# pxl-th/NNop.jl

Measured on AMD Instinct MI355X. Metric: attention TFLOPs/s + GB/s (fwd, fwd+bwd) at E=64,L=4096,H=4,B=4, higher is better.
Workload: dtype bf16; 1 GPU; C2: bf16 non-causal flash_attention forward, E=64 L=4096 QH=4 KH=4 B=4 per GPU; per_gpu_batch=4, global_batch=4, parallelism=dp1 over (batch, kv-head) slices, step=one nnop_fa_fwd call

## Files before the change

### nnop.jl_amd/csrc/fa_bwd_inst.hpp

```cpp
#pragma once
#include "fa_bwd.hpp"
#include "fa_bwd_w64.hpp"
#include "fa_launch.hpp"
#include "fa_generic.hpp"
#include <math.h>

namespace nnop {

template <typename T, int E> struct BwdCfg {
    static constexpr bool kF32 = sizeof(T) == 4;
    static constexpr int NW_KV = (kF32 && E > 128) ? (NNOP_F32_E256_FORM == 2 ? 4 : NNOP_F32_E256_FORM == 1 ? 2 : 1) : ((kF32 && E > 64 && !fa_bwd_f32_wide<T, E>()) || E > 128) ? 2 : 4;
    static constexpr int BQ    = (kF32 || E > 64) ? 32 : 64;
    static constexpr int NW_Q  = (kF32 && E > 128) ? (NNOP_F32_E256_FORM == 2 ? 4 : 1) : ((kF32 && E > 64 && !fa_bwd_f32_wide<T, E>()) || E > 128) ? 2 : 4;
    static constexpr bool kBig7 = !kF32 && E == 128;
    static constexpr bool kWide8 = !kF32 && E <= 64;
    static constexpr int BK    = (E > 64) ? 32 : 64;
};

static inline int bwd_causal_alt(const nnop_fa_desc& d, long long n_wg, long long cols, int rep, int n_blk, bool pair) {
    if (d.emb > 64 || pair) return 0;
    return causal_alt_run(d.causal != 0, n_wg, cols, rep, n_blk);
}

template <typename T, int E, int NW, int BQ, int MODE, bool WIN = false>
static int launch_dkdv(const nnop_fa_desc& d, const BwdParams& p, hipStream_t s) {
    constexpr int BM = bwd_base_mode(MODE);
    constexpr int lds = fa_bwd_dkdv_lds_bytes<T, E, NW, BQ, BM>() + (BM == 3 ? NW * PairTile<T>::kBytes : 0);
    static_assert(lds <= 160 * 1024, "LDS budget");
    auto kern = fa_bwd_dkdv_kernel<T, E, NW, BQ, MODE, WIN>;
    static unsigned long long lds_done = 0;
    if (ensure_dynamic_lds(kern, lds, &lds_done) != NNOP_OK) return NNOP_ERR_HIP;
    BwdParams pk = p;
    pk.n_blk = (d.kl + 32 * NW - 1) / (32 * NW);
    const long long n_wg = (long long)pk.n_blk * d.kh * d.batch;
    if (n_wg > 0x7fffffffLL) return NNOP_ERR_SHAPE;
    pk.n_wg = (int)n_wg;
    if (n_wg * fa_bwd_split<T, E>() > 0x7fffffffLL) return NNOP_ERR_SHAPE;
    pk.causal_alt = WIN ? 0 : bwd_causal_alt(d, n_wg, (long long)d.kh * d.batch, 1, pk.n_blk, BM >= 2);
    hipLaunchKernelGGL(kern, dim3((unsigned)(n_wg * fa_bwd_split<T, E>())), dim3(NW * 64), lds, s, pk);
    return NNOP_OK;
}

template <typename T, int E, int NW, int BK, int MODE, bool WIN = false>
static int launch_dq(const nnop_fa_desc& d, const BwdParams& p, hipStream_t s) {
    constexpr int BM = bwd_base_mode(MODE);
    constexpr int lds = fa_bwd_dq_lds_bytes<T, E, NW, BK, BM>() + (BM == 3 ? NW * PairTile<T>::kBytes : 0);
    static_assert(lds <= 160 * 1024, "LDS budget");
    auto kern = fa_bwd_dq_kernel<T, E, NW, BK, MODE, WIN>;
    static unsigned long long lds_done = 0;
    if (ensure_dynamic_lds(kern, lds, &lds_done) != NNOP_OK) return NNOP_ERR_HIP;
    BwdParams pq = p;
    pq.n_blk = (d.ql + 32 * NW - 1) / (32 * NW);
    const long long n_wg = (long long)pq.n_blk * d.qh * d.batch;
    if (n_wg > 0x7fffffffLL) return NNOP_ERR_SHAPE;
    pq.n_wg = (int)n_wg;
    if (n_wg * fa_bwd_split<T, E>() > 0x7fffffffLL) return NNOP_ERR_SHAPE;
    pq.causal_alt = WIN ? 0 : bwd_causal_alt(d, n_wg, (long long)d.qh * d.batch, d.qh / d.kh, pq.n_blk, BM >= 2);
    hipLaunchKernelGGL(kern, dim3((unsigned)(n_wg * fa_bwd_split<T, E>())), dim3(NW * 64), lds, s, pq);
    return NNOP_OK;
}

template <typename T, int E, int KIND, int MODE, int NARROW = 0>
static int launch_bwd_w64(const nnop_fa_desc& d, const BwdParams& p, hipStream_t s) {
    using SH = BwdW64Shape<E, KIND, NARROW>;
    constexpr int lds = fa_bwd_w64_lds_bytes<T, E, KIND, NARROW>(MODE != 0);
    static_assert(lds <= 160 * 1024, "LDS budget");
    auto kern = fa_bwd_w64_kernel<T, E, KIND, MODE, NARROW>;
    static unsigned long long lds_done = 0;
    if (ensure_dynamic_lds(kern, lds, &lds_done) != NNOP_OK) return NNOP_ERR_HIP;
    BwdParams pk = p;
    const int len = KIND == kBwdDQ ? d.ql : d.kl, hd = KIND == kBwdDQ ? d.qh : d.kh;
    pk.n_blk = (len + SH::WG_ROWS - 1) / SH::WG_ROWS;
    const long long n_wg = (long long)pk.n_blk * hd * d.batch;
    if (n_wg > 0x7fffffffLL) return NNOP_ERR_SHAPE;
    pk.n_wg = (int)n_wg;
    if (n_wg * SH::NSPLIT > 0x7fffffffLL) return NNOP_ERR_SHAPE;
    long long grid = n_wg * SH::NSPLIT;
    if constexpr (MODE == 1 && SH::NSPLIT == 1) {
        const bool pays = (d.causal && !p.kpad) || (KIND == kBwdDQ && !d.causal && p.kpad && hd % 8 == 0);
        const PersistList l = persist_list((long long)d.batch * hd, hd, pk.n_blk, tune_get(kTuneBwdPersist), pays);
        pk.persist = l.steps;
        pk.persist_hx = l.hx;
        if (l.steps > 0) grid = 256;
    }
    hipLaunchKernelGGL(kern, dim3((unsigned)grid), dim3(256), lds, s, pk);
    return NNOP_OK;
}
static inline bool bwd_w64_ok(const nnop_fa_desc& d, int kind) {
    if (d.dtype == NNOP_F32 || (d.emb != 64 && d.emb != 128 && d.emb != 256)) return false;
    const long long rb = 2LL * d.emb;
    if (kind == kBwdDKDV) {
        if ((long long)(d.qh / d.kh) * d.ql * rb >= (1LL << 32)) return false;
        if ((long long)bwd_rows_padded(d) * 32 >= (1LL << 32)) return false;
        return true;
    }
    return (long long)d.kl * rb < (1LL << 32) && d.kl <= 64 * kMaxMaskTiles;
}
static inline bool bwd_w64_narrow(const nnop_fa_desc& d, int kind) {
    if (d.emb != 64 && d.emb != 128) return false;
    const int knob = tune_get(kTuneBwdNarrow);
    if (knob >= 0) return knob != 0;
    const int len = kind == kBwdDQ ? d.ql : d.kl, hd = kind == kBwdDQ ? d.qh : d.kh;
    return small_grid_prefers_32_row_waves(len, (long long)hd * d.batch, d.causal != 0);
}
static inline int bwd_w64_forms(const nnop_fa_desc& d, bool has_pair, bool ws_aligned16, bool win_on, bool capped) {
    if (has_pair || win_on || capped) return 0;
    const int t = tune_get(kTuneBwdW64);
    const bool want_kv = t < 0 || t == 1 || t == 2 || t == 4, want_q = t < 0 || t == 1 || t == 3 || t == 4;
    return ((want_kv && ws_aligned16 && bwd_w64_ok(d, kBwdDKDV)) ? 1 : 0) | ((want_q && bwd_w64_ok(d, kBwdDQ)) ? 2 : 0);
}

static inline void bwd_params(BwdParams& p, const nnop_fa_desc& d, const BwdArgs& a) {
    p = BwdParams{};
    p.dq = a.dq; p.dk = a.dk; p.dv = a.dv; p.dpair = a.pair ? a.dpair : nullptr;
    p.d_o = a.d_o; p.o = a.o; p.ms = a.ms; p.ls = a.ls;
    p.q = a.q; p.k = a.k; p.v = a.v; p.pair = a.pair; p.kpad = a.kpad;
    p.nl = (float*)a.workspace;
    p.QL = d.ql; p.KL = d.kl; p.QH = d.qh; p.KH = d.kh; p.B = d.batch;
    p.causal = d.causal ? 1 : 0;
    p.scale = (float)(1.0 / sqrt((double)d.emb));
    p.win_left = a.win.left; p.win_right = a.win.right;
    if (a.softcap != 0.f) { const SoftcapK ck = softcap_k(1.0 / sqrt((double)d.emb), a.softcap); p.cap_ka = ck.ka; p.cap_kb = ck.kb; }
}

template <typename T, int E, int MODE, bool WIN = false>
static int launch_bwd_cfg(const nnop_fa_desc& d, const BwdArgs& a, hipStream_t s) {
    using C = BwdCfg<T, E>;
    BwdParams p;
    bwd_params(p, d, a);
    p.QLs = (d.ql + 63) & ~63;
    const long long n_rows = (long long)d.batch * d.qh * p.QLs;
    if (n_rows > 0x7fffffffLL) return NNOP_ERR_SHAPE;
    p.delta = p.nl + n_rows;
    p.rcf = (bwd_has_rcf(d) && ((uintptr_t)a.workspace & 15) == 0) ? (void*)(p.delta + n_rows) : nullptr;
    p.QLp = pair_pad(d.ql); p.KLp = pair_pad(d.kl);
    if constexpr (MODE == 3) {
        const size_t base = (bwd_workspace_bytes(d) + 255) & ~(size_t)255;
        const size_t one = (pair_scratch_elems(d) * sizeof(T) + 255) & ~(size_t)255;
        char* w = (char*)a.workspace + base;
        p.pair_a = w; p.dpair_s = w + one;
        const long long nblk = (long long)d.batch * (p.KLp / 32) * (p.QLp / 32);
        if (nblk > 0x7fffffffLL) return NNOP_ERR_SHAPE;
        PairPackParams pp{a.pair, (void*)p.pair_a, d.ql, d.kl, d.qh, d.batch, p.QLp, p.KLp, d.causal ? 1 : 0};
        hipLaunchKernelGGL((pair_pack_kernel<T>), dim3((unsigned)nblk), dim3(256), 1024 * d.qh * sizeof(T), s, pp);
    }

    const int stages = tune_get(kTuneBwdStages) < 0 ? 7 : tune_get(kTuneBwdStages);
    const int w64_forms = bwd_w64_forms(d, a.pair != nullptr, p.rcf != nullptr, a.win.on(), a.softcap != 0.f);
    const bool w64_kv = (w64_forms & 1) != 0, w64_q = (w64_forms & 2) != 0;
    p.fused = (w64_kv && w64_q && tune_get(kTuneBwdW64) != 4) ? 1 : 0;
    if ((stages & 1) && !p.fused) {
        const long long n_thr = n_rows * (E / 8);
        const long long grid = (n_thr + 255) / 256;
        if (grid > 0x7fffffffLL) return NNOP_ERR_SHAPE;
        hipLaunchKernelGGL((fa_bwd_pre_kernel<T, E>), dim3((unsigned)grid), dim3(256), 0, s, p, n_rows);
    }
    if (p.dpair && MODE != 3) {
        const size_t bytes = (size_t)d.batch * d.kl * d.ql * d.qh * sizeof(T);
        if (hipMemsetAsync(p.dpair, 0, bytes, s) != hipSuccess) { (void)hipGetLastError(); return NNOP_ERR_HIP; }
    }
    const int big_tune = tune_get(kTuneBwdBig7);
    const int big_thr = big_tune >= 0 ? big_tune : (d.causal ? 512 : 256);
    auto run_dkdv = [&]() -> int {
        if constexpr (WIN) return launch_dkdv<T, E, C::NW_KV, C::BQ, MODE, true>(d, p, s);
        else {
        int st = NNOP_OK;
        bool done = false;
        if constexpr (MODE <= 1 && sizeof(T) == 2 && (E == 64 || E == 128 || E == 256)) {
            if (w64_kv) {
                if constexpr (E != 256) {
                    if (bwd_w64_narrow(d, kBwdDKDV)) { st = launch_bwd_w64<T, E, kBwdDKDV, MODE, 1>(d, p, s); done = true; }
                }
                if (!done) { st = launch_bwd_w64<T, E, kBwdDKDV, MODE>(d, p, s); done = true; }
            }
        }
        if constexpr (C::kBig7) if (!done) {
            constexpr int NWB = fa_bwd_dkdv_kregs<T, E, MODE>() ? 8 : 7;
            const long long nb = (long long)((d.kl + 32 * NWB - 1) / (32 * NWB)) * d.kh * d.batch;
            if (nb >= big_thr) { st = launch_dkdv<T, E, NWB, C::BQ, MODE>(d, p, s); done = true; }
        }
        if constexpr (C::kWide8) if (!done) {
            const long long n8 = (long long)((d.kl + 255) / 256) * d.kh * d.batch;
            const int nw = tune_get(kTuneBwdNW);
            if (MODE != 2 && (nw == 8 || nw == 81 || (nw < 0 && !d.causal && n8 >= 256))) { st = launch_dkdv<T, E, 8, C::BQ, MODE>(d, p, s); done = true; }
        }
        if (!done) st = launch_dkdv<T, E, C::NW_KV, C::BQ, MODE>(d, p, s);
        return st;
        }
    };
    auto run_dq = [&]() -> int {
        if constexpr (WIN) return launch_dq<T, E, C::NW_Q, C::BK, MODE, true>(d, p, s);
        else {
        int st = NNOP_OK;
        bool done = false;
        if constexpr (MODE <= 1 && sizeof(T) == 2 && (E == 64 || E == 128 || E == 256)) {
            if (w64_q) {
                if constexpr (E != 256) {
                    if (bwd_w64_narrow(d, kBwdDQ)) {
                        if (MODE == 0 && (d.kl & 63) != 0) st = launch_bwd_w64<T, E, kBwdDQ, 1, 1>(d, p, s);
                        else st = launch_bwd_w64<T, E, kBwdDQ, MODE, 1>(d, p, s);
                        done = true;
                    }
                }
                if (!done) {
                    if (MODE == 0 && (d.kl & 31) != 0) st = launch_bwd_w64<T, E, kBwdDQ, 1>(d, p, s);
                    else st = launch_bwd_w64<T, E, kBwdDQ, MODE>(d, p, s);
                    done = true;
                }
            }
        }
        if constexpr (C::kBig7) if (!done) {
            constexpr int NWB = fa_bwd_dq_qregs<T, E, MODE>() ? 8 : 7;
            const long long nb = (long long)((d.ql + 32 * NWB - 1) / (32 * NWB)) * d.qh * d.batch;
            if (nb >= big_thr) { st = launch_dq<T, E, NWB, C::BK, MODE>(d, p, s); done = true; }
        }
        if constexpr (C::kWide8) if (!done) {
            const long long n8 = (long long)((d.ql + 255) / 256) * d.qh * d.batch;
            const int nw = tune_get(kTuneBwdNW);
            if (MODE != 2 && (nw == 8 || nw == 82 || (nw < 0 && !d.causal && n8 >= 256))) { st = launch_dq<T, E, 8, C::BK, MODE>(d, p, s); done = true; }
        }
        if (!done) st = launch_dq<T, E, C::NW_Q, C::BK, MODE>(d, p, s);
        return st;
        }
    };
    if (p.fused) {
        if (stages & 4) { const int st = run_dq(); if (st != NNOP_OK) return st; }
        if (stages & 2) { const int st = run_dkdv(); if (st != NNOP_OK) return st; }
    } else {
        if (stages & 2) { const int st = run_dkdv(); if (st != NNOP_OK) return st; }
        if (stages & 4) { const int st = run_dq(); if (st != NNOP_OK) return st; }
    }
    if constexpr (MODE == 3) {
        const long long nblk = (long long)d.batch * (p.KLp / 32) * (p.QLp / 32);
        PairUnpackParams up{a.dpair, p.dpair_s, a.kpad, d.ql, d.kl, d.qh, d.batch, p.QLp, p.KLp, d.causal ? 1 : 0,
                            PairTile<T>::kStoreLaneMajor ? 1 : 0};
        hipLaunchKernelGGL((dpair_unpack_kernel<T>), dim3((unsigned)nblk), dim3(256), 1024 * d.qh * sizeof(T), s, up);
    }
    return hipGetLastError() == hipSuccess ? NNOP_OK : NNOP_ERR_HIP;
}

template <typename T, int E>
static int launch_bwd_e(const nnop_fa_desc& d, const BwdArgs& a, hipStream_t s) {
    if (a.softcap != 0.f) {
        if constexpr (sizeof(T) == 4 && E == 256) return NNOP_ERR_EMB_UNSUPPORTED;
        else return a.pair ? launch_bwd_cfg<T, E, 2 | kBwdCap, true>(d, a, s) : launch_bwd_cfg<T, E, 1 | kBwdCap, true>(d, a, s);
    }
    if (a.win.on()) {
        if constexpr (sizeof(T) == 4 && E == 256) {
            if (a.pair) return NNOP_ERR_EMB_UNSUPPORTED;
            return launch_bwd_cfg<T, E, 1, true>(d, a, s);
        } else {
            return a.pair ? launch_bwd_cfg<T, E, 2, true>(d, a, s) : launch_bwd_cfg<T, E, 1, true>(d, a, s);
        }
    }
    if constexpr (sizeof(T) == 4 && E == 256) {
        if (a.pair) return NNOP_ERR_EMB_UNSUPPORTED;
        return (d.causal || a.kpad) ? launch_bwd_cfg<T, E, 1>(d, a, s) : launch_bwd_cfg<T, E, 0>(d, a, s);
    } else
    if (a.pair) {
        if (pair_staged_ok(d) && a.workspace_bytes >= bwd_workspace_bytes_pair(d) && bwd_workspace_bytes_pair(d) > bwd_workspace_bytes(d) &&
            ((uintptr_t)a.workspace & 15) == 0)
            return launch_bwd_cfg<T, E, 3>(d, a, s);
        return launch_bwd_cfg<T, E, 2>(d, a, s);
    }
    if (d.causal || a.kpad) return launch_bwd_cfg<T, E, 1>(d, a, s);
    return launch_bwd_cfg<T, E, 0>(d, a, s);
}

template <typename T> static int launch_bwd_generic(const nnop_fa_desc& d, const BwdArgs& a, hipStream_t s) {
    BwdParams p;
    bwd_params(p, d, a);
    const long long n_rows = (long long)d.batch * d.qh * d.ql, n_krows = (long long)d.batch * d.kh * d.kl;
    p.QLs = d.ql;
    p.delta = p.nl + n_rows;
    const long long gq = (n_rows + 3) / 4, gk = (n_krows + 3) / 4;
    if (gq > 0x7fffffffLL || gk > 0x7fffffffLL) return NNOP_ERR_SHAPE;
    if (p.dpair) {
        const size_t bytes = (size_t)d.batch * d.kl * d.ql * d.qh * sizeof(T);
        if (hipMemsetAsync(p.dpair, 0, bytes, s) != hipSuccess) { (void)hipGetLastError(); return NNOP_ERR_HIP; }
    }
    hipLaunchKernelGGL((fa_bwd_generic_pre_kernel<T>), dim3((unsigned)gq), dim3(256), 0, s, p, d.emb, n_rows);
    const bool cap = a.softcap != 0.f;
    hipLaunchKernelGGL((cap ? fa_bwd_generic_dq_kernel<T, true> : fa_bwd_generic_dq_kernel<T, false>), dim3((unsigned)gq), dim3(256), 0, s, p, d.emb, n_rows);
    hipLaunchKernelGGL((cap ? fa_bwd_generic_dkdv_kernel<T, true> : fa_bwd_generic_dkdv_kernel<T, false>), dim3((unsigned)gk), dim3(256), 0, s, p, d.emb, n_krows);
    return hipGetLastError() == hipSuccess ? NNOP_OK : NNOP_ERR_HIP;
}

template <typename T> int launch_bwd(const nnop_fa_desc& d, const BwdArgs& a, hipStream_t s) {
    if constexpr (sizeof(T) == 2) {
        if (d.emb == 256) return launch_bwd_e<T, 256>(d, a, s);
    } else {
        if (d.emb == 256 && !a.pair && a.softcap == 0.f) return launch_bwd_e<T, 256>(d, a, s);
    }
    if (emb_generic(d.emb)) return launch_bwd_generic<T>(d, a, s);
    switch (d.emb) {
        case 16:  return launch_bwd_e<T, 16>(d, a, s);
        case 32:  return launch_bwd_e<T, 32>(d, a, s);
        case 64:  return launch_bwd_e<T, 64>(d, a, s);
        case 128: return launch_bwd_e<T, 128>(d, a, s);
        default:  return NNOP_ERR_EMB_UNSUPPORTED;
    }
}

}
```

### nnop.jl_amd/csrc/fa_bwd_w64.hpp

```cpp
#pragma once
#include "fa_bwd.hpp"
#include "fa_fwd_w64.hpp"

#if !defined(NNOP_DEV_BUILD)
#undef NNOP_BW64_STAMP
#endif
#ifndef NNOP_BW64_STAMP
#define NNOP_BW64_STAMP 0
#endif
#ifndef NNOP_BW64_LAG
#define NNOP_BW64_LAG 3
#endif
#ifndef NNOP_BW64_PF
#define NNOP_BW64_PF 3
#endif

namespace nnop {

enum : int { kBwdDKDV = 0, kBwdDQ = 1 };

template <typename T, int E> struct DualImg {
    static_assert(sizeof(T) == 2 && (E == 64 || E == 128 || E == 256), "16-bit element types, E = 64, 128 or 256");
    static constexpr int kRowBytes = 2 * E;
    static constexpr int bytes(int rows) { return rows * kRowBytes; }
    NNOP_DEV static constexpr int xor_of(int row) {
        if constexpr (E >= 128) return ((row & 3) << 2) | ((row >> 2) & 3);
        else return (((row >> 1) & 1) << 2) | (((row >> 3) & 1) << 1) | ((row >> 2) & 1);
    }
    NNOP_DEV static int src_of(int o) {
        const int row = o / kRowBytes, phys = (o % kRowBytes) >> 4;
        return row * kRowBytes + ((phys ^ xor_of(row)) << 4);
    }
    NNOP_DEV static int row_lane_base(int lane) {
        const int r = lane & 31, h = lane >> 5;
        return r * kRowBytes + ((xor_of(r) ^ h) << 4);
    }
    NNOP_DEV static int col_lane_base(int lane) {
        const int h = lane >> 5, g1 = (lane >> 4) & 1, q = (lane >> 2) & 3, p = lane & 3;
        const int qx = E >= 128 ? q : (q >> 1);
        return (4 * h + q) * kRowBytes + 16 * (4 * qx + ((2 * g1 + (p >> 1)) ^ h)) + 8 * (p & 1);
    }
};

template <int E, int KIND, int NARROW = 0> struct BwdW64Shape {
    static constexpr bool kDQ = KIND == kBwdDQ;
    static_assert(!NARROW || E == 64 || E == 128, "narrow form: E = 64 / 128");
    static constexpr bool kVLds = !kDQ && E == 128 && !NARROW;
    static constexpr int ZS = (E == 256 || NARROW) ? 1 : ((kDQ || E == 64 || kVLds) ? 2 : 1);
    static constexpr int ZT = E == 256 ? 1 : 2 / ZS;
    static constexpr int NSPLIT = (!kDQ && E == 256) ? 2 : 1;
    static constexpr int NYP = kDQ ? 1 : 2;
    static constexpr int KS = E / 16, EB = E / 32, EBA = EB / NSPLIT;
    static constexpr int NEL = 16 * ZS * ZT;
    static constexpr int RT = 32 * ZT, SW = 32 * ZS, RB = 2 * E;
    static constexpr int IMG = RT * RB;
    static constexpr int RCM = kDQ ? 0 : 1;
    static constexpr int RCB = kDQ ? 0 : RT * 32;
    static constexpr int SLOT = 2 * IMG + RCB, NS = 4;
    static constexpr int NJ = IMG / 4096;
    static constexpr int NPB = 2 * NJ + RCM;
    static constexpr int NFY = NYP * 2 * ZT * EBA, NFX = 2 * ZT * KS, NF = NFY + NFX;
    static constexpr int TB = ZS * (KS + RCM);
    static constexpr int NY = NFY * ZS, NX = 2 * ZT * TB, NSLOT = NY + NX;
    static constexpr int WG_ROWS = 4 * SW;
    static constexpr bool kBases = E == 64 && !kDQ;
    static constexpr int VIMG = kVLds ? WG_ROWS * RB : 0;
    static constexpr int NVB = kVLds ? ZS * KS : 0, PFB = 3, RFB = 4;
    static constexpr int vb_slot(int b) { return NY + TB + ZS * RCM + b; }
    static_assert(IMG % 4096 == 0 && NJ >= 1 && NJ <= 4, "four waves x NJ pieces = one image; 12-bit immediate");
    static_assert(SLOT % (RB > 256 ? RB : 256) == 0, "XOR-addressed fragment reads: slot bases aligned to a row / 256 bytes");
};
template <typename T, int E, int KIND, int NARROW = 0> constexpr int fa_bwd_w64_lds_bytes(bool masked) {
    using SH = BwdW64Shape<E, KIND, NARROW>;
    return SH::NS * SH::SLOT + SH::VIMG + (masked ? (SH::kDQ ? 16 + 8 * kMaxMaskTiles : 16) : 0);
}

template <int E, int KIND, bool MASKED, int LAG, int PF, int NARROW = 0> struct BwdW64Plan {
    using SH = BwdW64Shape<E, KIND, NARROW>;
    static constexpr int NSLOT = SH::NSLOT, NEL = SH::NEL, NITEM = NEL + NEL + NEL / 2;
    static constexpr int BAR_SLOT = (SH::NFY - PF) * SH::ZS;
    int kind[NITEM] = {};
    int el[NITEM] = {};
    int it_end[NSLOT] = {};
    int cost[NSLOT] = {};
    int cap = 0;

    static constexpr bool x_is_rc(int j) { return SH::RCM && (j % SH::TB) / SH::ZS == 0; }
    static constexpr int x_frag(int j) { return (j / SH::TB) * SH::KS + (j % SH::TB) / SH::ZS - SH::RCM; }
    static constexpr int rc_slot(int tq) { return SH::NY + tq * SH::TB; }
    static constexpr int rc_read_slot(int tq) { return rc_slot(tq) - 3 > BAR_SLOT ? rc_slot(tq) - 3 : BAR_SLOT; }
    static constexpr int dma_slot(int d) { return BAR_SLOT + 1 + 2 * d; }
    static constexpr int slot_frag(int s) {
        if (s < SH::NY) return s % SH::ZS == 0 ? s / SH::ZS : -1;
        const int j = s - SH::NY;
        if (x_is_rc(j) || j % SH::ZS != 0) return -1;
        return SH::NFY + x_frag(j);
    }
    static constexpr int pre_cost(int s) {
        int c = 0;
        if (s == BAR_SLOT) c += 8;
        const int f = slot_frag(s % NSLOT);
        if (f >= 0) c += ((f + PF) % SH::NF < SH::NFY ? 24 : 16) + 2 - (SH::kBases ? 4 : 0);
        if (s == NSLOT) c += 24 + 18 + 16 + (MASKED ? 30 : 0);
        return c;
    }
    static constexpr int post_cost(int s) {
        int c = 0;
        for (int tq = 0; tq < 2 * SH::ZT * SH::RCM; ++tq)
            if (s == rc_read_slot(tq)) c += 12;
        if (s == BAR_SLOT + 1) c += SH::kDQ ? 24 : 60;
        if (SH::kBases && s == 1) c += 4 * SH::KS;
        if (SH::kBases && s == SH::NY + 1) c += 8 * SH::EBA;
        for (int b = 0; b < SH::NVB; ++b)
            if (s == SH::vb_slot(b) - SH::PFB) c += 16;
        for (int d = 0; d < SH::NPB; ++d)
            if (s == dma_slot(d)) c += 40 + ((d % SH::NJ == 0 || d >= 2 * SH::NJ) ? 14 : 0);
        return c;
    }
    static constexpr int item_cost(int k) { return k == 0 ? 12 : (k == 1 ? 4 : 4 * SH::NYP); }
    constexpr void list() {
        int n = 0;
        for (int st = 0; st < NEL + LAG; ++st) {
            if (st < NEL) { kind[n] = 0; el[n++] = st; }
            const int m = st - LAG;
            if (m >= 0) {
                kind[n] = 1; el[n++] = m;
                if (m & 1) { kind[n] = 2; el[n++] = m; }
            }
        }
    }
    constexpr bool fill(int budget) {
        int n = 0;
        for (int g = 0; g < NSLOT; ++g) {
            int used = post_cost(g) + pre_cost(g + 1);
            while (n < NITEM && used + item_cost(kind[n]) <= budget && !(g == 0 && kind[n] != 0)) used += item_cost(kind[n++]);
            it_end[g] = n;
            cost[g] = used;
        }
        cap = budget;
        return n == NITEM;
    }
    static constexpr BwdW64Plan make() {
        BwdW64Plan pl{};
        pl.list();
        for (int b = 8; b <= 200; b += 2)
            if (pl.fill(b)) break;
        return pl;
    }
};

template <typename T, int EB> NNOP_DEV void store_acc_row16(T* rowp, f32x16 (&acc)[EB], float mul, int h, bool ok) {
#pragma unroll
    for (int eb = 0; eb < EB; ++eb) {
        acc_after_fence(acc[eb]);
        uint32_t pk[4][2];
#pragma unroll
        for (int g = 0; g < 4; ++g) {
            typedef T t4 __attribute__((ext_vector_type(4)));
            const f32x4 w = {acc[eb][4 * g] * mul, acc[eb][4 * g + 1] * mul, acc[eb][4 * g + 2] * mul, acc[eb][4 * g + 3] * mul};
            const u32x2 u = __builtin_bit_cast(u32x2, __builtin_convertvector(w, t4));
            pk[g][0] = u[0];
            pk[g][1] = u[1];
        }
#pragma unroll
        for (int g = 0; g < 4; g += 2) {
            const auto s0 = __builtin_amdgcn_permlane32_swap(pk[g][0], pk[g + 1][0], false, false);
            const auto s1 = __builtin_amdgcn_permlane32_swap(pk[g][1], pk[g + 1][1], false, false);
            const u32x4 lo = {s0[0], s1[0], s0[1], s1[1]};
            if (ok) *reinterpret_cast<u32x4*>(rowp + 32 * eb + 8 * g + 8 * h) = lo;
        }
    }
}

template <typename T, int E, int KIND, int MODE, int NARROW = 0>
__global__ __launch_bounds__(256, 1) void fa_bwd_w64_kernel(const BwdParams p_arg) {
    using SH = BwdW64Shape<E, KIND, NARROW>;
    using frag_t = typename Elem<T>::frag;
    using Img = DualImg<T, E>;
    using MM = MfmaAsm<T>;
    constexpr bool kDQ = SH::kDQ, kGeneral = MODE != 0;
    constexpr int ZS = SH::ZS, ZT = SH::ZT, NYP = SH::NYP, KS = SH::KS, EB = SH::EBA;
    constexpr int RT = SH::RT, SW = SH::SW, RB = SH::RB, IMG = SH::IMG, SLOT = SH::SLOT, NS = SH::NS, NJ = SH::NJ, NPB = SH::NPB;
    constexpr int NFY = SH::NFY, NF = SH::NF, NY = SH::NY, NX = SH::NX, NSLOT = SH::NSLOT;
    constexpr int PF = NNOP_BW64_PF, RF = 4, LAG = NNOP_BW64_LAG;
    static_assert(NF % RF == 0 && PF < RF && PF < NFY, "static fragment ring; the barrier sits inside phase Y");

    extern __shared__ __attribute__((aligned(16))) char smem[];
#if NNOP_BW64_STAMP
    uint64_t stamp[6];
    stamp[0] = __builtin_amdgcn_s_memtime();
    stamp[1] = __builtin_amdgcn_s_memrealtime();
#endif
    const int wave = __builtin_amdgcn_readfirstlane((int)threadIdx.x >> 6);

    constexpr bool kPersist = kGeneral && SH::NSPLIT == 1;
    const int n_steps_pers = (kPersist && p_arg.persist > 0) ? p_arg.persist : 1;
    for (int pstep = 0; pstep < n_steps_pers; ++pstep) {
    int lane0 = 0;
    if constexpr (kPersist) asm volatile("s_mov_b32 %0, 0" : "=s"(lane0));
    const int lane = kPersist ? (int)__builtin_amdgcn_mbcnt_hi(~0u, __builtin_amdgcn_mbcnt_lo(~0u, (uint32_t)lane0)) : ((int)threadIdx.x & 63);
    const int tid = wave * 64 + lane;
    const int r = lane & 31, h = lane >> 5;
    BwdParams p_blk;
    if constexpr (!kPersist) p_blk = p_arg;
    if constexpr (kPersist) {
        p_blk.dpair = nullptr; p_blk.pair = nullptr; p_blk.pair_a = nullptr; p_blk.dpair_s = nullptr; p_blk.QLp = 0; p_blk.KLp = 0;
        typedef const BwdParams __attribute__((address_space(4))) * params_cp;
        params_cp pp = (params_cp)__builtin_amdgcn_kernarg_segment_ptr();
        asm volatile("" : "+s"(pp));
        p_blk.dq = pp->dq; p_blk.dk = pp->dk; p_blk.dv = pp->dv; p_blk.d_o = pp->d_o; p_blk.o = pp->o; p_blk.ms = pp->ms; p_blk.ls = pp->ls;
        p_blk.q = pp->q; p_blk.k = pp->k; p_blk.v = pp->v; p_blk.kpad = pp->kpad; p_blk.nl = pp->nl; p_blk.delta = pp->delta;
        p_blk.QL = pp->QL; p_blk.KL = pp->KL; p_blk.QH = pp->QH; p_blk.KH = pp->KH; p_blk.B = pp->B; p_blk.causal = pp->causal;
        p_blk.QLs = pp->QLs; p_blk.fused = pp->fused; p_blk.rcf = pp->rcf; p_blk.n_blk = pp->n_blk; p_blk.n_wg = pp->n_wg;
        p_blk.scale = pp->scale; p_blk.persist = pp->persist; p_blk.persist_hx = pp->persist_hx;
    }
    const BwdParams& p = p_blk;
    const float c2 = p.scale * kLog2e;
    const int rep = p.QH / p.KH;
    int pers_col = 0, pers_k = 0;
    if (kPersist && p.persist > 0) {
        const int c = (int)blockIdx.x >> 3;
        const int pos = 32 * pstep + ((pstep & 1) ? 31 - c : c);
        pers_col = pos / p.n_blk;
        pers_k = pos - pers_col * p.n_blk;
    }

    int b, kvh, bh_s;
    int s0wg;
    int SL, TL;
    int heads, u0 = 0, nps;
    if constexpr (kDQ) {
        int blk;
        if (kPersist && p.persist > 0) {
            blk = p.n_blk - 1 - pers_k;
            if (p.persist_hx > 0) bh_s = (pers_col / p.persist_hx) * p.QH + ((int)blockIdx.x & 7) * p.persist_hx + pers_col % p.persist_hx;
            else bh_s = ((int)blockIdx.x & 7) * ((p.B * p.QH) >> 3) + pers_col;
        } else {
            const int lin = xcd_remap_chunked((int)blockIdx.x, p.n_wg, p.n_blk * rep);
            blk = lin % p.n_blk;
            bh_s = lin / p.n_blk;
            if (kGeneral && p.causal) blk = p.n_blk - 1 - blk;
        }
        b = bh_s / p.QH;
        kvh = (bh_s - b * p.QH) / rep;
        s0wg = blk * SH::WG_ROWS;
        SL = p.QL; TL = p.KL; heads = 1;
        nps = (TL + RT - 1) / RT;
        if (kGeneral && p.causal) {
            int last = s0wg + SH::WG_ROWS - 1;
            if (last > SL - 1) last = SL - 1;
            const int t_c = last / RT + 1;
            if (t_c < nps) nps = t_c;
        }
    } else {
        int blk;
        if (kPersist && p.persist > 0) {
            blk = pers_k;
            if (p.persist_hx > 0) bh_s = (pers_col / p.persist_hx) * p.KH + ((int)blockIdx.x & 7) * p.persist_hx + pers_col % p.persist_hx;
            else bh_s = ((int)blockIdx.x & 7) * ((p.B * p.KH) >> 3) + pers_col;
        } else {
            const int lin = xcd_remap_chunked((int)blockIdx.x % p.n_wg, p.n_wg, p.n_blk);
            blk = lin % p.n_blk;
            bh_s = lin / p.n_blk;
        }
        b = bh_s / p.KH;
        kvh = bh_s - b * p.KH;
        s0wg = blk * SH::WG_ROWS;
        SL = p.KL; TL = p.QL; heads = rep;
        const int nst = (TL + RT - 1) / RT;
        if (kGeneral && p.causal) u0 = s0wg / RT < nst ? s0wg / RT : nst;
        nps = nst - u0;
    }
    const int esplit = SH::NSPLIT > 1 ? (int)blockIdx.x / p.n_wg : 0;
    const int s0w = s0wg + wave * SW;
    int sidx[ZS], sidx_c[ZS];
#pragma unroll
    for (int zs = 0; zs < ZS; ++zs) {
        sidx[zs] = s0w + 32 * zs + r;
        sidx_c[zs] = sidx[zs] < SL ? sidx[zs] : SL - 1;
    }

    const T* __restrict__ b1p;
    const T* __restrict__ b2p;
    const char* __restrict__ t1p;
    const char* __restrict__ t2p;
    uint32_t t_bytes;
    if constexpr (kDQ) {
        b1p = (const T*)p.q + (size_t)bh_s * p.QL * E;
        b2p = (const T*)p.d_o + (size_t)bh_s * p.QL * E;
        t1p = (const char*)((const T*)p.k + (size_t)(b * p.KH + kvh) * p.KL * E);
        t2p = (const char*)((const T*)p.v + (size_t)(b * p.KH + kvh) * p.KL * E);
        t_bytes = (uint32_t)p.KL * (uint32_t)RB;
    } else {
        b1p = (const T*)p.k + (size_t)bh_s * p.KL * E;
        b2p = (const T*)p.v + (size_t)bh_s * p.KL * E;
        const size_t g0 = (size_t)(b * p.QH + kvh * rep) * p.QL * E;
        t1p = (const char*)((const T*)p.q + g0);
        t2p = (const char*)((const T*)p.d_o + g0);
        t_bytes = (uint32_t)rep * (uint32_t)p.QL * (uint32_t)RB;
    }
    const int U = heads * nps;

    const uint8_t* __restrict__ mp = kGeneral && p.kpad ? p.kpad + (size_t)b * p.KL : nullptr;
    bool svalid[ZS];
#pragma unroll
    for (int zs = 0; zs < ZS; ++zs) svalid[zs] = sidx[zs] < SL;
    uint64_t* const vbits = reinterpret_cast<uint64_t*>(smem + NS * SLOT + SH::VIMG + 16);
    int n_steps = U;
    if constexpr (kGeneral && !kDQ) {
        if (mp) {
            bool any = false;
#pragma unroll
            for (int zs = 0; zs < ZS; ++zs) {
                if (svalid[zs]) svalid[zs] = mp[sidx[zs]] != 0;
                any = any || svalid[zs];
            }
            int* flag = reinterpret_cast<int*>(smem + NS * SLOT + SH::VIMG);
            if (tid == 0) *flag = 0;
            __syncthreads();
            if (any) *flag = 1;
            __syncthreads();
            if (*flag == 0) n_steps = 0;
        }
    }
    if constexpr (kGeneral && kDQ) {
        int* slot = reinterpret_cast<int*>(smem + NS * SLOT + SH::VIMG);
        const int nk = n_steps * RT < p.KL ? n_steps * RT : p.KL;
        if (mp) {
            const int last = kpad_scan(mp, p.KL, nk, vbits, kMaxMaskTiles, slot, tid, 256);
            const int t_m = last / RT + 1;
            if (t_m < n_steps) n_steps = t_m;
        } else {
            for (int w = tid; w * 64 < nk; w += 256) {
                const int left = p.KL - w * 64;
                vbits[w] = left >= 64 ? ~0ull : ((1ull << left) - 1ull);
            }
            __syncthreads();
        }
    }

    n_steps = __builtin_amdgcn_readfirstlane(n_steps);

    float rc_nl[ZS], rc_nd[ZS];
    frag_t rc_do[kDQ ? ZS : 1][kDQ ? KS : 1], rc_o[kDQ ? ZS : 1][kDQ ? KS : 1];
    T rc_m[ZS], rc_l[ZS];
    if constexpr (kDQ) {
#pragma unroll
        for (int zs = 0; zs < ZS; ++zs) {
            const bool in = sidx[zs] < SL;
            const size_t row = (size_t)bh_s * p.QL + sidx_c[zs];
            const T* drow = (const T*)p.d_o + row * E;
#pragma unroll
            for (int ks = 0; ks < KS; ++ks) rc_do[zs][ks] = *reinterpret_cast<const frag_t*>(drow + 16 * ks + 8 * h);
            if (p.fused) {
                const T* orow = (const T*)p.o + row * E;
#pragma unroll
                for (int ks = 0; ks < KS; ++ks) rc_o[zs][ks] = *reinterpret_cast<const frag_t*>(orow + 16 * ks + 8 * h);
                rc_m[zs] = ((const T*)p.ms)[row];
                rc_l[zs] = ((const T*)p.ls)[row];
            } else {
                const size_t ro = (size_t)bh_s * p.QLs + sidx_c[zs];
                rc_nl[zs] = in ? p.nl[ro] : -INFINITY;
                rc_nd[zs] = in ? p.delta[ro] : 0.f;
            }
        }
    }
    auto finish_rc = [&]() {
        if constexpr (kDQ) {
            if (!p.fused) return;
#pragma unroll
            for (int zs = 0; zs < ZS; ++zs) {
                float part = 0.f;
#pragma unroll
                for (int ks = 0; ks < KS; ++ks)
#pragma unroll
                    for (int j = 0; j < 8; ++j) part += to_f32(rc_do[zs][ks][j]) * to_f32(rc_o[zs][ks][j]);
                const float dl = half_swap_sum(part);
                const float m = to_f32(rc_m[zs]), l = to_f32(rc_l[zs]);
                float nlv = -(m * kLog2e + __builtin_amdgcn_logf(l)) / c2;
                float ndv = -dl;
                if (!(l > 0.f) || !(nlv == nlv) || m == -INFINITY) { nlv = -INFINITY; ndv = 0.f; }
                if (!(sidx[zs] < SL)) { nlv = -INFINITY; ndv = 0.f; }
                if (p.rcf && sidx[zs] < p.QLs && h == 0) {
                    typedef T t8 __attribute__((ext_vector_type(8)));
                    t8* dst = reinterpret_cast<t8*>(p.rcf) + 2 * ((size_t)bh_s * p.QLs + sidx[zs]);
                    dst[0] = rc_split3<T>(nlv);
                    dst[1] = rc_split3<T>(ndv);
                }
                rc_nl[zs] = nlv;
                rc_nd[zs] = ndv;
            }
        }
    };
    if (n_steps == 0) finish_rc();
    f32x16 acc[NYP][ZS][EB];
#pragma unroll
    for (int y = 0; y < NYP; ++y)
#pragma unroll
        for (int zs = 0; zs < ZS; ++zs)
#pragma unroll
            for (int eb = 0; eb < EB; ++eb) {
#pragma unroll
                for (int i = 0; i < 16; ++i) acc[y][zs][eb][i] = 0.f;
                asm volatile("" : "+a"(acc[y][zs][eb]));
            }

    if (n_steps > 0) {
        const uint32_t lds0 = (uint32_t)(uintptr_t)smem;
        if ((TL & (RT - 1)) != 0) {
            for (int i = tid * 16; i < NS * SLOT; i += 256 * 16) *reinterpret_cast<u32x4*>(smem + i) = u32x4{0, 0, 0, 0};
            __syncthreads();
        }
        uint32_t voff[NJ];
#pragma unroll
        for (int j = 0; j < NJ; ++j) voff[j] = (uint32_t)(Img::src_of((wave * NJ + j) * 1024 + lane * 16) - j * 1024);
        const uint32_t wave_off = (uint32_t)(wave * NJ * 1024);
        const u32x4 rs1 = make_rsrc(t1p, t_bytes), rs2 = make_rsrc(t2p, t_bytes);
        u32x4 rsc = rs1;
        uint32_t rc_voff = 0;
        if constexpr (!kDQ) {
            rsc = make_rsrc(p.rcf, (uint32_t)((size_t)p.B * p.QH * p.QLs * 32));
            rc_voff = (uint32_t)lane * 16u + (uint32_t)((wave % (RT / 32)) * 1024);
        }
        const uint32_t rc_dst_off = (uint32_t)(2 * IMG) + (uint32_t)((wave % (RT / 32 > 0 ? RT / 32 : 1)) * 1024);
        int d_s = 0;
        uint32_t d_off = (uint32_t)u0 * (uint32_t)(RT * RB);
        uint32_t d_rc = kDQ ? 0u : ((uint32_t)(b * p.QH + kvh * rep) * (uint32_t)p.QLs + (uint32_t)(u0 * RT)) * 32u;
        const uint32_t jump_off = ((uint32_t)p.QL - (uint32_t)((nps - 1) * RT)) * (uint32_t)RB;
        const uint32_t jump_rc = ((uint32_t)p.QLs - (uint32_t)((nps - 1) * RT)) * 32u;
        auto advance_dma = [&]() {
            if constexpr (kDQ) {
                d_off += (uint32_t)(RT * RB);
            } else {
                const int s1 = d_s + 1;
                const bool wrap = s1 == nps;
                d_s = wrap ? 0 : s1;
                d_off += wrap ? jump_off : (uint32_t)(RT * RB);
                d_rc += wrap ? jump_rc : (uint32_t)(RT * 32);
            }
        };
        auto issue_step = [&](uint32_t slot) {
            static_for<NJ>([&](auto jc) { constexpr int j = decltype(jc)::value; dma_piece<j, j == 0>(rs1, voff[j], d_off, slot); });
            static_for<NJ>([&](auto jc) { constexpr int j = decltype(jc)::value; dma_piece<j, j == 0>(rs2, voff[j], d_off, slot + IMG); });
            if constexpr (!kDQ) dma_piece<0, true>(rsc, rc_voff, d_rc, slot - wave_off + rc_dst_off);
        };
        uint32_t sM = lds0 + wave_off, sX = sM + SLOT, sF = sM + 2 * SLOT, sD = sM + 3 * SLOT, sY = sM;
        auto rotate_slots = [&]() { sY = sM; sM = sX; sX = sF; sF = sD; sD = sY; };

        constexpr bool kVLds = SH::kVLds;
        frag_t b1[ZS][KS], b2[kVLds ? 1 : ZS][kVLds ? 1 : KS];
#pragma unroll
        for (int zs = 0; zs < ZS; ++zs)
#pragma unroll
            for (int ks = 0; ks < KS; ++ks) {
                if constexpr (kVLds) {
                    b1[zs][ks] = *reinterpret_cast<const frag_t*>(b1p + (size_t)sidx_c[zs] * E + 16 * ks + 8 * h);
                } else {
                    b1[zs][ks] = load_q_frag<frag_t>(b1p + (size_t)sidx_c[zs] * E + 16 * ks + 8 * h);
                    if constexpr (kDQ) b2[zs][ks] = rc_do[zs][ks];
                    else b2[zs][ks] = load_q_frag<frag_t>(b2p + (size_t)sidx_c[zs] * E + 16 * ks + 8 * h);
                }
            }
        const uint32_t vimg0 = lds0 + (uint32_t)(NS * SLOT);
        if constexpr (kVLds) {
            const u32x4 rsv = make_rsrc(b2p, (uint32_t)SL * (uint32_t)RB);
            const uint32_t vsoff = (uint32_t)s0wg * (uint32_t)RB;
            static_for<16>([&](auto jc) {
                constexpr int j = decltype(jc)::value;
                const uint32_t vo = (uint32_t)(Img::src_of((wave * 16 + j) * 1024 + lane * 16) - (j & 3) * 1024);
                dma_piece<(j & 3), (j & 3) == 0>(rsv, vo, vsoff, vimg0 + (uint32_t)(wave * 16384 + (j >> 2) * 4096));
            });
        }
        issue_step(sM);
        advance_dma();
        issue_step(sX);
        advance_dma();
        issue_step(sF);
        advance_dma();
        finish_rc();
        float nl2[ZS];
        f32x16 ndl[ZS];
        if constexpr (kDQ) {
#pragma unroll
            for (int zs = 0; zs < ZS; ++zs) {
                nl2[zs] = rc_nl[zs] * c2;
#pragma unroll
                for (int i = 0; i < 16; ++i) ndl[zs][i] = rc_nd[zs];
            }
            if constexpr (ZS == 2) fence_valu_operand(ndl[0], ndl[1]);
            else asm volatile("s_nop 1" : "+v"(ndl[0]));
        }
        constexpr bool kBonesV = E == 256 || kVLds;
        frag_t bones;
        if constexpr (!kDQ) {
#pragma unroll
            for (int j = 0; j < 8; ++j) bones[j] = from_f32<T>((h == 0 && j < 3) ? 1.0f : 0.0f);
            if constexpr (kBonesV) asm volatile("s_nop 1" : "+v"(bones));
            else asm volatile("s_nop 1" : "+a"(bones));
        }
        auto rc_tile = [&](frag_t rc) -> f32x16 { if constexpr (kBonesV) return MM::qk_first_v(rc, bones); else return MM::qk_first(rc, bones); };

        f32x16 sA[ZS][ZT], dA[ZS][ZT], sB[ZS][ZT], dB[ZS][ZT];
        u32x4 fA[NYP][ZS][2 * ZT], fB[NYP][ZS][2 * ZT];
#pragma unroll
        for (int y = 0; y < NYP; ++y)
#pragma unroll
            for (int zs = 0; zs < ZS; ++zs)
#pragma unroll
                for (int kk = 0; kk < 2 * ZT; ++kk) { fA[y][zs][kk] = u32x4{0, 0, 0, 0}; fB[y][zs][kk] = u32x4{0, 0, 0, 0}; }

        typedef __attribute__((address_space(3))) const frag_t* lds_frag_p;
        typedef __attribute__((address_space(3))) s16x4* lds_tr_p;
        const uint32_t row_lane = (uint32_t)Img::row_lane_base(lane) - wave_off;
        const uint32_t col_lane = (uint32_t)Img::col_lane_base(lane) + (uint32_t)(esplit * EB * 64) - wave_off;
        const uint32_t rc_lane0 = (uint32_t)(2 * IMG + r * 32 + 16 * h) - wave_off;
        const uint32_t rc_lane1 = (uint32_t)(2 * IMG + r * 32 + 16) - wave_off;
        auto opaque = [](uint32_t x) { asm volatile("" : "+v"(x)); return x; };
        auto pin = [](auto& x) { asm volatile("" : "+v"(x)); };
        auto read_row = [&](uint32_t ra, int g) -> frag_t {
            const int prod = g / (ZT * KS), zt = (g / KS) % ZT, ks = g % KS;
            return *(lds_frag_p)(uintptr_t)((ra ^ (uint32_t)(ks << 5)) + (uint32_t)(prod * IMG + zt * 32 * RB));
        };
        auto read_col = [&](uint32_t ca, int f) -> frag_t {
            const int y = f / (2 * ZT * EB), kk = (f / EB) % (2 * ZT), eb = f % EB;
            const int img = kDQ ? 0 : (y == 0 ? IMG : 0);
            const s16x4 a = __builtin_amdgcn_ds_read_tr16_b64_v4i16((lds_tr_p)(uintptr_t)((ca ^ (uint32_t)(eb << 6)) + (uint32_t)(img + 16 * kk * RB)));
            const s16x4 c = __builtin_amdgcn_ds_read_tr16_b64_v4i16((lds_tr_p)(uintptr_t)((ca ^ (uint32_t)((eb << 6) | 32)) + (uint32_t)(img + (16 * kk + 8) * RB)));
            typedef short s16x8 __attribute__((ext_vector_type(8)));
            const s16x8 v8 = {a[0], a[1], a[2], a[3], c[0], c[1], c[2], c[3]};
            return __builtin_bit_cast(frag_t, v8);
        };
        auto read_row_b = [&](const uint32_t (&rb)[KS], int g) -> frag_t {
            const int prod = g / (ZT * KS), zt = (g / KS) % ZT, ks = g % KS;
            return *(lds_frag_p)(uintptr_t)(rb[ks] + (uint32_t)(prod * IMG + zt * 32 * RB));
        };
        auto read_col_b = [&](const uint32_t (&cb)[2 * EB], int f) -> frag_t {
            const int y = f / (2 * ZT * EB), kk = (f / EB) % (2 * ZT), eb = f % EB;
            const int img = kDQ ? 0 : (y == 0 ? IMG : 0);
            const s16x4 a = __builtin_amdgcn_ds_read_tr16_b64_v4i16((lds_tr_p)(uintptr_t)(cb[2 * eb] + (uint32_t)(img + 16 * kk * RB)));
            const s16x4 c = __builtin_amdgcn_ds_read_tr16_b64_v4i16((lds_tr_p)(uintptr_t)(cb[2 * eb + 1] + (uint32_t)(img + (16 * kk + 8) * RB)));
            typedef short s16x8 __attribute__((ext_vector_type(8)));
            const s16x8 v8 = {a[0], a[1], a[2], a[3], c[0], c[1], c[2], c[3]};
            return __builtin_bit_cast(frag_t, v8);
        };
        const uint32_t v_lane = vimg0 + (uint32_t)(wave * 64 * RB + Img::row_lane_base(lane));
        auto read_vb = [&](int b) -> frag_t {
            const int ks = b / ZS, zs = b % ZS;
            return *(lds_frag_p)(uintptr_t)((v_lane ^ (uint32_t)(ks << 5)) + (uint32_t)(zs * 32 * RB));
        };
        auto read_rcf = [&](uint32_t rca, int zt) -> frag_t { return *(lds_frag_p)(uintptr_t)(rca + (uint32_t)(zt * 1024)); };

        uint64_t vword_next = 0;
        auto vword_fetch = [&](int u) { const int w = (u * RT) >> 6; vword_next = vbits[w < kMaxMaskTiles ? w : kMaxMaskTiles - 1]; };
        using vword_t = std::conditional_t<(kDQ && RT == 64), uint64_t, uint32_t>;
        constexpr vword_t kAllValid = ~(vword_t)0;
        auto vword_take = [&](int u) -> vword_t {
            const uint64_t w = ((uint64_t)(uint32_t)__builtin_amdgcn_readfirstlane((uint32_t)(vword_next >> 32)) << 32) |
                               (uint64_t)(uint32_t)__builtin_amdgcn_readfirstlane((uint32_t)vword_next);
            return (vword_t)(w >> ((u * RT) & 63));
        };
        auto apply_mask = [&](f32x16 (&s)[ZS][ZT], int t0, vword_t valid) {
#pragma unroll
            for (int zs = 0; zs < ZS; ++zs)
#pragma unroll
                for (int zt = 0; zt < ZT; ++zt) {
                    uint32_t m;
                    if constexpr (kDQ) {
                        const int lim = (p.causal ? sidx[zs] : 0x3fffffff) - t0 - 32 * zt - 4 * h;
                        const uint32_t cm = lim >= 31 ? ~0u : (lim < 0 ? 0u : ((2u << lim) - 1u));
                        m = (uint32_t)(valid >> (32 * zt + 4 * h)) & cm;
                    } else {
                        const int lim = sidx[zs] - t0 - 32 * zt - 4 * h;
                        m = lim <= 0 ? ~0u : (lim >= 32 ? 0u : ~((1u << lim) - 1u));
                    }
#pragma unroll
                    for (int i = 0; i < 16; ++i) {
                        const int lr = (i & 3) + 8 * (i >> 2);
                        s[zs][zt][i] = ((m >> lr) & 1u) ? s[zs][zt][i] : -INFINITY;
                    }
                }
        };
        int c_s = 0;
        auto step_t0 = [&]() -> int { return (u0 + c_s) * RT; };
        auto step_needs_mask = [&](int t0, vword_t valid) -> bool {
            if constexpr (kDQ) return valid != kAllValid || (p.causal && t0 + RT - 1 > s0w);
            else return p.causal && t0 < s0w + SW - 1;
        };

        if constexpr (kVLds) {
#pragma unroll
            for (int zs = 0; zs < ZS; ++zs)
#pragma unroll
                for (int ks = 0; ks < KS; ++ks) landed(b1[zs][ks]);
            asm volatile("s_waitcnt vmcnt(%c[nfl])\n\ts_barrier" :: [nfl] "n"(2 * NPB) : "memory");
        } else if constexpr (KS == 16) {
            static_assert(ZS == 1, "");
            asm volatile("s_waitcnt vmcnt(%c[nfl])\n\ts_barrier"
                         : "+a"(b1[0][0]), "+a"(b1[0][1]), "+a"(b1[0][2]), "+a"(b1[0][3]), "+a"(b1[0][4]), "+a"(b1[0][5]), "+a"(b1[0][6]), "+a"(b1[0][7])
                         : [nfl] "n"(2 * NPB) : "memory");
            asm volatile("" : "+a"(b1[0][8]), "+a"(b1[0][9]), "+a"(b1[0][10]), "+a"(b1[0][11]), "+a"(b1[0][12]), "+a"(b1[0][13]), "+a"(b1[0][14]), "+a"(b1[0][15]) :: "memory");
            asm volatile("" : "+a"(b2[0][0]), "+a"(b2[0][1]), "+a"(b2[0][2]), "+a"(b2[0][3]), "+a"(b2[0][4]), "+a"(b2[0][5]), "+a"(b2[0][6]), "+a"(b2[0][7]) :: "memory");
            asm volatile("" : "+a"(b2[0][8]), "+a"(b2[0][9]), "+a"(b2[0][10]), "+a"(b2[0][11]), "+a"(b2[0][12]), "+a"(b2[0][13]), "+a"(b2[0][14]), "+a"(b2[0][15]) :: "memory");
        } else if constexpr (KS == 8 && ZS == 2) {
            asm volatile("s_waitcnt vmcnt(%c[nfl])\n\ts_barrier"
                         : "+a"(b1[0][0]), "+a"(b1[0][1]), "+a"(b1[0][2]), "+a"(b1[0][3]), "+a"(b1[0][4]), "+a"(b1[0][5]), "+a"(b1[0][6]), "+a"(b1[0][7]),
                           "+a"(b1[1][0]), "+a"(b1[1][1]), "+a"(b1[1][2]), "+a"(b1[1][3]), "+a"(b1[1][4]), "+a"(b1[1][5]), "+a"(b1[1][6]), "+a"(b1[1][7])
                         : [nfl] "n"(2 * NPB) : "memory");
            asm volatile(""
                         : "+a"(b2[0][0]), "+a"(b2[0][1]), "+a"(b2[0][2]), "+a"(b2[0][3]), "+a"(b2[0][4]), "+a"(b2[0][5]), "+a"(b2[0][6]), "+a"(b2[0][7]),
                           "+a"(b2[1][0]), "+a"(b2[1][1]), "+a"(b2[1][2]), "+a"(b2[1][3]), "+a"(b2[1][4]), "+a"(b2[1][5]), "+a"(b2[1][6]), "+a"(b2[1][7])
                         :: "memory");
        } else if constexpr (KS == 8) {
            asm volatile("s_waitcnt vmcnt(%c[nfl])\n\ts_barrier"
                         : "+a"(b1[0][0]), "+a"(b1[0][1]), "+a"(b1[0][2]), "+a"(b1[0][3]), "+a"(b1[0][4]), "+a"(b1[0][5]), "+a"(b1[0][6]), "+a"(b1[0][7]),
                           "+a"(b2[0][0]), "+a"(b2[0][1]), "+a"(b2[0][2]), "+a"(b2[0][3]), "+a"(b2[0][4]), "+a"(b2[0][5]), "+a"(b2[0][6]), "+a"(b2[0][7])
                         : [nfl] "n"(2 * NPB) : "memory");
        } else if constexpr (KS == 4 && ZS == 1) {
            asm volatile("s_waitcnt vmcnt(%c[nfl])\n\ts_barrier"
                         : "+a"(b1[0][0]), "+a"(b1[0][1]), "+a"(b1[0][2]), "+a"(b1[0][3]), "+a"(b2[0][0]), "+a"(b2[0][1]), "+a"(b2[0][2]), "+a"(b2[0][3])
                         : [nfl] "n"(2 * NPB) : "memory");
        } else {
            static_assert(KS == 4 && ZS == 2, "");
            asm volatile("s_waitcnt vmcnt(%c[nfl])\n\ts_barrier"
                         : "+a"(b1[0][0]), "+a"(b1[0][1]), "+a"(b1[0][2]), "+a"(b1[0][3]), "+a"(b1[1][0]), "+a"(b1[1][1]), "+a"(b1[1][2]), "+a"(b1[1][3]),
                           "+a"(b2[0][0]), "+a"(b2[0][1]), "+a"(b2[0][2]), "+a"(b2[0][3]), "+a"(b2[1][0]), "+a"(b2[1][1]), "+a"(b2[1][2]), "+a"(b2[1][3])
                         : [nfl] "n"(2 * NPB) : "memory");
        }

        {
            const uint32_t ra = opaque(sM + row_lane);
            const uint32_t rca[2] = {opaque(sM + rc_lane0), opaque(sM + rc_lane1)};
#pragma unroll
            for (int prod = 0; prod < 2; ++prod)
#pragma unroll
                for (int zt = 0; zt < ZT; ++zt) {
                    if constexpr (!kDQ) {
                        const frag_t rc = read_rcf(rca[prod], zt);
#pragma unroll
                        for (int zs = 0; zs < ZS; ++zs) (prod ? dA : sA)[zs][zt] = rc_tile(rc);
                    }
#pragma unroll
                    for (int ks = 0; ks < KS; ++ks) {
                        const frag_t a = read_row(ra, (prod * ZT + zt) * KS + ks);
#pragma unroll
                        for (int zs = 0; zs < ZS; ++zs) {
                            f32x16& d = (prod ? dA : sA)[zs][zt];
                            if constexpr (kVLds) {
                                const frag_t bq = prod ? read_vb(ks * ZS + zs) : b1[zs][ks];
                                MM::qk_acc_v(d, a, bq);
                            } else {
                                const frag_t& bq = (prod ? b2 : b1)[zs][ks];
                                if (kDQ && ks == 0) d = prod ? MM::qk_init(a, bq, ndl[zs]) : MM::qk_first(a, bq);
                                else MM::qk_acc(d, a, bq);
                            }
                        }
                    }
                }
            if constexpr (ZS == 2) {
                fence_mfma_result(sA[0][0], sA[1][0], dA[0][0], dA[1][0]);
            } else if constexpr (ZT == 2) {
                fence_mfma_result(sA[0][0], sA[0][1], dA[0][0], dA[0][1]);
            } else {
                asm volatile(NNOP_FENCE_128 : "+v"(sA[0][0]), "+v"(dA[0][0]));
            }
        }
        if constexpr (kGeneral && kDQ) vword_fetch(0);

        frag_t fr[RF];
        {
            const uint32_t ca0 = opaque(sY + col_lane);
#pragma unroll
            for (int f = 0; f < PF; ++f) fr[f] = read_col(ca0, f);
        }

        constexpr bool kBases = SH::kBases;
        uint32_t cbase[2 * EB], rbase[KS];
        auto set_cbase = [&](uint32_t slot) {
            const uint32_t ca = opaque(slot + col_lane);
#pragma unroll
            for (int j = 0; j < 2 * EB; ++j) { cbase[j] = ca ^ (uint32_t)(((j >> 1) << 6) | ((j & 1) << 5)); pin(cbase[j]); }
        };
        if constexpr (kBases) set_cbase(sY);

        using Plan = BwdW64Plan<E, KIND, kGeneral, LAG, PF, NARROW>;
        auto iteration = [&](int u, f32x16 (&sc)[ZS][ZT], f32x16 (&dc)[ZS][ZT], f32x16 (&sn)[ZS][ZT], f32x16 (&dn)[ZS][ZT],
                             u32x4 (&fw)[NYP][ZS][2 * ZT], u32x4 (&fp)[NYP][ZS][2 * ZT]) {
            constexpr Plan plan = Plan::make();
            static_assert(plan.it_end[NSLOT - 1] == Plan::NITEM, "every item placed");
            static_assert(Plan::dma_slot(NPB - 1) < NSLOT, "the DMA batch fits behind the barrier");
            if constexpr (kGeneral) {
                const int t0 = step_t0();
                vword_t valid = kAllValid;
                if constexpr (kDQ) {
                    valid = vword_take(u);
                    vword_fetch(u + 1);
                }
                if (__builtin_expect(step_needs_mask(t0, valid), 0)) apply_mask(sc, t0, valid);
            }
            const uint32_t cimg = opaque(sY + col_lane);
            const uint32_t cimg2 = opaque(sM + col_lane);
            const uint32_t rimg = opaque(sX + row_lane);
            uint32_t rcimg[2] = {0, 0};
            if constexpr (!kDQ) { rcimg[0] = opaque(sX + rc_lane0); rcimg[1] = opaque(sX + rc_lane1); }
            frag_t rcf[2 * ZT];
            frag_t vb[kVLds ? SH::RFB : 1];
            uint32_t dst = 0, soff = 0, srow = 0;

            auto item = [&](auto kc) {
                constexpr int k = decltype(kc)::value, kind = plan.kind[k], n = plan.el[k];
                constexpr int t = n >> 4, zs = ZS == 2 ? t : 0, zt = ZS == 2 ? 0 : t, i = n & 15;
                if constexpr (kind == 0) {
                    float x;
                    if constexpr (kDQ) x = __builtin_fmaf(sc[zs][zt][i], c2, nl2[zs]);
                    else x = sc[zs][zt][i] * c2;
                    float e = fast_exp2(x);
                    pin(e);
                    sc[zs][zt][i] = e;
                } else if constexpr (kind == 1) {
                    float ds = sc[zs][zt][i] * dc[zs][zt][i];
                    pin(ds);
                    dc[zs][zt][i] = ds;
                } else {
                    typedef T t2 __attribute__((ext_vector_type(2)));
                    constexpr int kk = 2 * zt + (i >> 3), w = (i & 7) >> 1;
                    if constexpr (!kDQ) {
                        const f32x2 pw = {sc[zs][zt][i - 1], sc[zs][zt][i]};
                        uint32_t word2 = __builtin_bit_cast(uint32_t, __builtin_convertvector(pw, t2));
                        pin(word2);
                        fw[0][zs][kk][w] = word2;
                    }
                    const f32x2 dsw = {dc[zs][zt][i - 1], dc[zs][zt][i]};
                    uint32_t word = __builtin_bit_cast(uint32_t, __builtin_convertvector(dsw, t2));
                    pin(word);
                    fw[NYP - 1][zs][kk][w] = word;
                }
            };
            auto movable = [&](auto sc_) {
                constexpr int sl = decltype(sc_)::value;
                constexpr int k0 = sl ? plan.it_end[sl - 1] : 0, k1 = plan.it_end[sl];
                static_for<k1 - k0>([&](auto dk_) { item(std::integral_constant<int, k0 + decltype(dk_)::value>{}); });
            };
            auto read_ahead = [&](auto fc) {
                constexpr int g = decltype(fc)::value + PF;
                if constexpr (kBases) {
                    if constexpr (g < NFY) fr[g % RF] = read_col_b(cbase, g);
                    else if constexpr (g < NF) fr[g % RF] = read_row_b(rbase, g - NFY);
                    else fr[g % RF] = read_col_b(cbase, g - NF);
                } else {
                    if constexpr (g < NFY) fr[g % RF] = read_col(cimg, g);
                    else if constexpr (g < NF) fr[g % RF] = read_row(rimg, g - NFY);
                    else fr[g % RF] = read_col(cimg2, g - NF);
                }
            };

            static_for<NSLOT>([&](auto ic) {
                constexpr int i = decltype(ic)::value;
                constexpr int f = Plan::slot_frag(i);
                if constexpr (i == Plan::BAR_SLOT) {
                    static_assert(NPB <= 15, "vmcnt literal");
                    asm volatile("s_waitcnt vmcnt(%0)\n\ts_barrier" :: "n"(NPB) : "memory");
                }
                if constexpr (f >= 0) read_ahead(std::integral_constant<int, f>{});
                if constexpr (i < NY) {
                    constexpr int fy = i / ZS, zs = i % ZS;
                    constexpr int y = fy / (2 * ZT * EB), kk = (fy / EB) % (2 * ZT), eb = fy % EB;
                    MM::pv_acc(acc[y][zs][eb], fr[fy % RF], __builtin_bit_cast(frag_t, fp[y][zs][kk]));
                } else {
                    constexpr int j = i - NY, tq = j / SH::TB, prod = tq / ZT, zt = tq % ZT, zs = (j % SH::TB) % ZS;
                    f32x16& d = (prod ? dn : sn)[zs][zt];
                    if constexpr (Plan::x_is_rc(j)) {
                        d = rc_tile(rcf[tq]);
                    } else {
                        constexpr int g = Plan::x_frag(j), ks = g % KS;
                        if constexpr (kVLds) {
                            if constexpr (prod == 0) MM::qk_acc_v(d, fr[(NFY + g) % RF], b1[zs][ks]);
                            else MM::qk_acc_v(d, fr[(NFY + g) % RF], vb[(ks * ZS + zs) % SH::RFB]);
                        } else {
                            const frag_t& bq = (prod ? b2 : b1)[zs][ks];
                            if constexpr (kDQ && ks == 0) d = prod ? MM::qk_init(fr[(NFY + g) % RF], bq, ndl[zs]) : MM::qk_first(fr[(NFY + g) % RF], bq);
                            else MM::qk_acc(d, fr[(NFY + g) % RF], bq);
                        }
                    }
                }
                __builtin_amdgcn_sched_barrier(0);
                if constexpr (!kDQ) {
                    static_for<2 * ZT>([&](auto tc) {
                        constexpr int tq = decltype(tc)::value;
                        if constexpr (i == Plan::rc_read_slot(tq)) rcf[tq] = read_rcf(rcimg[tq / ZT], tq % ZT);
                    });
                }
                if constexpr (kVLds) {
                    static_for<SH::NVB>([&](auto bc) {
                        constexpr int b = decltype(bc)::value;
                        if constexpr (i == SH::vb_slot(b) - SH::PFB) vb[b % SH::RFB] = read_vb(b);
                    });
                }
                if constexpr (kBases && i == 1) {
#pragma unroll
                    for (int ks = 0; ks < KS; ++ks) { rbase[ks] = rimg ^ (uint32_t)(ks << 5); pin(rbase[ks]); }
                }
                if constexpr (kBases && i == NY + 1) set_cbase(sM);
                if constexpr (i == Plan::BAR_SLOT + 1) {
                    dst = sD;
                    soff = d_off;
                    srow = d_rc;
                    advance_dma();
                    asm volatile("" : "+s"(d_off));
                }
                static_for<NPB>([&](auto dc_) {
                    constexpr int d = decltype(dc_)::value;
                    if constexpr (i == Plan::dma_slot(d)) {
                        if constexpr (d < NJ) dma_piece<d, d == 0>(rs1, voff[d < NJ ? d : 0], soff, dst);
                        else if constexpr (d < 2 * NJ) dma_piece<d - NJ, d == NJ>(rs2, voff[d < 2 * NJ ? d - NJ : 0], soff, dst + IMG);
                        else dma_piece<0, true>(rsc, rc_voff, srow, dst - wave_off + rc_dst_off);
                    }
                });
                movable(std::integral_constant<int, i>{});
                __builtin_amdgcn_sched_barrier(0);
            });
            rotate_slots();
            if constexpr (kGeneral) {
                if constexpr (kDQ) ++c_s;
                else { if (++c_s == nps) c_s = 0; }
            }
        };

        auto leave_fence = []() { asm volatile(NNOP_FENCE_128 ::: "memory"); __builtin_amdgcn_sched_barrier(0); };
#if NNOP_BW64_STAMP
        stamp[2] = __builtin_amdgcn_s_memtime();
        stamp[3] = __builtin_amdgcn_s_memrealtime();
#endif
        int n_live = n_steps;
        if constexpr (kDQ && kGeneral) {
            if (p.causal) {
                const int t_w = (s0w + SW - 1) / RT + 1;
                if (t_w < n_live) n_live = t_w;
            }
        }
        int u = 0;
        const int n_it = n_live + 1;
        if (n_it >= 2) {
            for (;;) {
                iteration(u, sA, dA, sB, dB, fA, fB);
                iteration(u + 1, sB, dB, sA, dA, fB, fA);
                u += 2;
                if (u + 1 >= n_it) {
                    leave_fence();
                    break;
                }
            }
        }
        if (u < n_it) {
            iteration(u, sA, dA, sB, dB, fA, fB);
            leave_fence();
            ++u;
        }
        if constexpr (kDQ && kGeneral) {
            for (; u <= n_steps; ++u) {
                asm volatile("s_waitcnt vmcnt(%0)\n\ts_barrier" :: "n"(NPB) : "memory");
                issue_step(sD);
                advance_dma();
                rotate_slots();
            }
        }
        asm volatile("s_waitcnt vmcnt(0)" ::: "memory");
#if NNOP_BW64_STAMP
        stamp[4] = __builtin_amdgcn_s_memtime();
        stamp[5] = __builtin_amdgcn_s_memrealtime();
#endif
    }

    fence_acc_result(acc[0][0][0]);
    int lane1 = 0;
    if constexpr (kPersist) asm volatile("s_mov_b32 %0, 0" : "=s"(lane1));
    const int lane_e = kPersist ? (int)__builtin_amdgcn_mbcnt_hi(~0u, __builtin_amdgcn_mbcnt_lo(~0u, (uint32_t)lane1)) : lane;
    const int h_e = lane_e >> 5;
#pragma unroll
    for (int zs = 0; zs < ZS; ++zs) {
        const int sidx_e = kPersist ? s0w + 32 * zs + (lane_e & 31) : sidx[zs];
        const int sidx_ce = sidx_e < SL ? sidx_e : SL - 1;
        const bool in = sidx_e < SL;
        if constexpr (kDQ) {
            T* row = (T*)p.dq + ((size_t)bh_s * p.QL + sidx_ce) * E + esplit * EB * 32;
            store_acc_row16<T, EB>(row, acc[0][zs], p.scale, h_e, in);
        } else {
            if constexpr (kGeneral) {
                if (!svalid[zs]) {
#pragma unroll
                    for (int y = 0; y < NYP; ++y)
#pragma unroll
                        for (int eb = 0; eb < EB; ++eb) {
                            acc_after_fence(acc[y][zs][eb]);
#pragma unroll
                            for (int i = 0; i < 16; ++i) acc[y][zs][eb][i] = 0.f;
                        }
                }
            }
            const size_t ro = ((size_t)bh_s * p.KL + sidx_ce) * E + esplit * EB * 32;
            store_acc_row16<T, EB>((T*)p.dv + ro, acc[0][zs], 1.0f, h_e, in);
            store_acc_row16<T, EB>((T*)p.dk + ro, acc[1][zs], p.scale, h_e, in);
        }
    }
#if NNOP_BW64_STAMP
    if (tid == 0) {
        uint64_t* dbg = kDQ ? reinterpret_cast<uint64_t*>((T*)p.dq + ((size_t)bh_s * p.QL + s0w) * E)
                            : reinterpret_cast<uint64_t*>((T*)p.dk + ((size_t)bh_s * p.KL + s0w) * E);
        for (int i = 0; i < 6; ++i) dbg[i] = stamp[i];
        dbg[6] = (uint64_t)n_steps;
    }
#endif
    if (pstep + 1 < n_steps_pers) __syncthreads();
    }
}

}
```

Baseline: 984.8 TFLOP/s.

## Use compile-time LDS ring slots and an MHA-specialised dK/dV backward kernel

Turns the four-slot LDS ring of the w64 backward kernel from rotating runtime registers into compile-time slot indices. The main loop is unrolled four times so fragment reads and buffer-to-LDS DMA can use immediate offsets from precomputed per-lane base registers. Adds a one-head variant for the dK/dV pass when query heads equal kv heads, which removes the per-step wrap logic, and retunes the scheduling cost model. The aim is fewer address computations and scalar ALU work per step, at the cost of more code size and register pressure.

```diff
diff --git a/nnop.jl_amd/csrc/fa_bwd_inst.hpp b/nnop.jl_amd/csrc/fa_bwd_inst.hpp
--- a/nnop.jl_amd/csrc/fa_bwd_inst.hpp
+++ b/nnop.jl_amd/csrc/fa_bwd_inst.hpp
@@ -60,12 +60,18 @@
     return NNOP_OK;
 }
 
-template <typename T, int E, int KIND, int MODE, int NARROW = 0>
+template <typename T, int E, int KIND, int MODE, int NARROW = 0, bool ONEHEAD = false>
 static int launch_bwd_w64(const nnop_fa_desc& d, const BwdParams& p, hipStream_t s) {
     using SH = BwdW64Shape<E, KIND, NARROW>;
+    if constexpr (!ONEHEAD && KIND == kBwdDKDV && E == 64 && NARROW == 0) {
+        if (d.qh == d.kh) return launch_bwd_w64<T, E, KIND, MODE, NARROW, true>(d, p, s);
+    }
     constexpr int lds = fa_bwd_w64_lds_bytes<T, E, KIND, NARROW>(MODE != 0);
     static_assert(lds <= 160 * 1024, "LDS budget");
-    auto kern = fa_bwd_w64_kernel<T, E, KIND, MODE, NARROW>;
+    auto kern = [] {
+        if constexpr (ONEHEAD) return fa_bwd_w64_mha_kernel<T, E, KIND, MODE, NARROW>;
+        else return fa_bwd_w64_kernel<T, E, KIND, MODE, NARROW>;
+    }();
     static unsigned long long lds_done = 0;
     if (ensure_dynamic_lds(kern, lds, &lds_done) != NNOP_OK) return NNOP_ERR_HIP;
     BwdParams pk = p;
diff --git a/nnop.jl_amd/csrc/fa_bwd_w64.hpp b/nnop.jl_amd/csrc/fa_bwd_w64.hpp
--- a/nnop.jl_amd/csrc/fa_bwd_w64.hpp
+++ b/nnop.jl_amd/csrc/fa_bwd_w64.hpp
@@ -18,6 +18,7 @@
 namespace nnop {
 
 enum : int { kBwdDKDV = 0, kBwdDQ = 1 };
+template <int V> using w64_ic = std::integral_constant<int, V>;
 
 template <typename T, int E> struct DualImg {
     static_assert(sizeof(T) == 2 && (E == 64 || E == 128 || E == 256), "16-bit element types, E = 64, 128 or 256");
@@ -63,7 +64,12 @@
     static constexpr int TB = ZS * (KS + RCM);
     static constexpr int NY = NFY * ZS, NX = 2 * ZT * TB, NSLOT = NY + NX;
     static constexpr int WG_ROWS = 4 * SW;
-    static constexpr bool kBases = E == 64 && !kDQ;
+    static constexpr int kMaxTileOff = (kDQ ? 0 : IMG) + (16 * (2 * ZT - 1) + 8) * RB > IMG + (ZT - 1) * 32 * RB
+                                           ? (kDQ ? 0 : IMG) + (16 * (2 * ZT - 1) + 8) * RB : IMG + (ZT - 1) * 32 * RB;
+    static constexpr int SB = 3 * SLOT + kMaxTileOff < 65536 ? 4 : (SLOT + kMaxTileOff < 65536 ? 2 : 1);
+    static constexpr int NBS = NS / SB;
+    static_assert((SB - 1) * SLOT + kMaxTileOff < 65536 && kMaxTileOff < 65536, "16-bit DS offset field");
+    static constexpr bool kBases = E == 64;
     static constexpr int VIMG = kVLds ? WG_ROWS * RB : 0;
     static constexpr int NVB = kVLds ? ZS * KS : 0, PFB = 3, RFB = 4;
     static constexpr int vb_slot(int b) { return NY + TB + ZS * RCM + b; }
@@ -75,7 +81,7 @@
     return SH::NS * SH::SLOT + SH::VIMG + (masked ? (SH::kDQ ? 16 + 8 * kMaxMaskTiles : 16) : 0);
 }
 
-template <int E, int KIND, bool MASKED, int LAG, int PF, int NARROW = 0> struct BwdW64Plan {
+template <int E, int KIND, bool MASKED, int LAG, int PF, int NARROW = 0, bool ONEHEAD = false, bool CS = true> struct BwdW64Plan {
     using SH = BwdW64Shape<E, KIND, NARROW>;
     static constexpr int NSLOT = SH::NSLOT, NEL = SH::NEL, NITEM = NEL + NEL + NEL / 2;
     static constexpr int BAR_SLOT = (SH::NFY - PF) * SH::ZS;
@@ -100,21 +106,20 @@
         int c = 0;
         if (s == BAR_SLOT) c += 8;
         const int f = slot_frag(s % NSLOT);
-        if (f >= 0) c += ((f + PF) % SH::NF < SH::NFY ? 24 : 16) + 2 - (SH::kBases ? 4 : 0);
-        if (s == NSLOT) c += 24 + 18 + 16 + (MASKED ? 30 : 0);
+        if (f >= 0) c += ((f + PF) % SH::NF < SH::NFY ? 24 : 16) + 2 - (SH::kBases && CS ? 4 : 0);
+        if (s == NSLOT) c += (CS ? 12 : 24 + 18 + 16) + (MASKED ? 30 : 0);
         return c;
     }
     static constexpr int post_cost(int s) {
         int c = 0;
         for (int tq = 0; tq < 2 * SH::ZT * SH::RCM; ++tq)
             if (s == rc_read_slot(tq)) c += 12;
-        if (s == BAR_SLOT + 1) c += SH::kDQ ? 24 : 60;
-        if (SH::kBases && s == 1) c += 4 * SH::KS;
-        if (SH::kBases && s == SH::NY + 1) c += 8 * SH::EBA;
+        if (CS && s == dma_slot(SH::NPB - 1)) c += SH::kDQ ? 6 : (ONEHEAD ? 12 : 42);
+        if (!CS && s == BAR_SLOT + 1) c += SH::kDQ ? 24 : 60;
         for (int b = 0; b < SH::NVB; ++b)
             if (s == SH::vb_slot(b) - SH::PFB) c += 16;
         for (int d = 0; d < SH::NPB; ++d)
-            if (s == dma_slot(d)) c += 40 + ((d % SH::NJ == 0 || d >= 2 * SH::NJ) ? 14 : 0);
+            if (s == dma_slot(d)) c += 40 + ((d % SH::NJ == 0 || d >= 2 * SH::NJ) ? (CS ? 8 : 14) : 0);
         return c;
     }
     static constexpr int item_cost(int k) { return k == 0 ? 12 : (k == 1 ? 4 : 4 * SH::NYP); }
@@ -129,11 +134,12 @@
             }
         }
     }
-    constexpr bool fill(int budget) {
+    constexpr bool fill(int budget, int n_low = 0) {
         int n = 0;
         for (int g = 0; g < NSLOT; ++g) {
             int used = post_cost(g) + pre_cost(g + 1);
-            while (n < NITEM && used + item_cost(kind[n]) <= budget && !(g == 0 && kind[n] != 0)) used += item_cost(kind[n++]);
+            const int bg = g < n_low ? budget - 2 : budget;
+            while (n < NITEM && used + item_cost(kind[n]) <= bg && !(g == 0 && kind[n] != 0)) used += item_cost(kind[n++]);
             it_end[g] = n;
             cost[g] = used;
         }
@@ -143,8 +149,11 @@
     static constexpr BwdW64Plan make() {
         BwdW64Plan pl{};
         pl.list();
-        for (int b = 8; b <= 200; b += 2)
-            if (pl.fill(b)) break;
+        int b = 8;
+        while (b <= 200 && !pl.fill(b)) b += 2;
+        int n_low = CS ? NSLOT : 0;
+        while (n_low > 0 && !pl.fill(b, n_low)) --n_low;
+        if (n_low == 0) pl.fill(b);
         return pl;
     }
 };
@@ -172,8 +181,17 @@
     }
 }
 
-template <typename T, int E, int KIND, int MODE, int NARROW = 0>
-__global__ __launch_bounds__(256, 1) void fa_bwd_w64_kernel(const BwdParams p_arg) {
+template <int J, bool FIRST, int OFF> NNOP_DEV void dma_piece_at(u32x4 rsrc, uint32_t voff, uint32_t soff, uint32_t ring) {
+    if constexpr (FIRST && OFF != 0)
+        asm volatile("s_add_u32 m0, %3, %5\n\ts_nop 0\n\tbuffer_load_dwordx4 %0, %1, %2 offen offset:%4 lds"
+                     :: "v"(voff), "s"(rsrc), "s"(soff), "s"(ring), "n"(J * 1024), "n"(OFF) : "memory", "scc");
+    else
+        dma_piece<J, FIRST>(rsrc, voff, soff, ring);
+}
+
+template <typename T, int E, int KIND, int MODE, int NARROW, bool ONEHEAD>
+NNOP_DEV void fa_bwd_w64_body(const BwdParams& p_arg) {
+    static_assert(!ONEHEAD || KIND == kBwdDKDV, "the dQ pass streams one kv-head: it has no wrap");
     using SH = BwdW64Shape<E, KIND, NARROW>;
     using frag_t = typename Elem<T>::frag;
     using Img = DualImg<T, E>;
@@ -183,6 +201,7 @@
     constexpr int RT = SH::RT, SW = SH::SW, RB = SH::RB, IMG = SH::IMG, SLOT = SH::SLOT, NS = SH::NS, NJ = SH::NJ, NPB = SH::NPB;
     constexpr int NFY = SH::NFY, NF = SH::NF, NY = SH::NY, NX = SH::NX, NSLOT = SH::NSLOT;
     constexpr int PF = NNOP_BW64_PF, RF = 4, LAG = NNOP_BW64_LAG;
+    constexpr bool kConstSlots = !(!NARROW && ((E == 128 && (!kDQ || kGeneral)) || (E == 256 && kDQ && kGeneral)));
     static_assert(NF % RF == 0 && PF < RF && PF < NFY, "static fragment ring; the barrier sits inside phase Y");
 
     extern __shared__ __attribute__((aligned(16))) char smem[];
@@ -407,8 +426,9 @@
 
     if (n_steps > 0) {
         const uint32_t lds0 = (uint32_t)(uintptr_t)smem;
-        if ((TL & (RT - 1)) != 0) {
-            for (int i = tid * 16; i < NS * SLOT; i += 256 * 16) *reinterpret_cast<u32x4*>(smem + i) = u32x4{0, 0, 0, 0};
+        {
+            const int z0 = (TL & (RT - 1)) != 0 ? 0 : (NS - 1) * SLOT;
+            for (int i = z0 + tid * 16; i < NS * SLOT; i += 256 * 16) *reinterpret_cast<u32x4*>(smem + i) = u32x4{0, 0, 0, 0};
             __syncthreads();
         }
         uint32_t voff[NJ];
@@ -423,14 +443,18 @@
             rc_voff = (uint32_t)lane * 16u + (uint32_t)((wave % (RT / 32)) * 1024);
         }
         const uint32_t rc_dst_off = (uint32_t)(2 * IMG) + (uint32_t)((wave % (RT / 32 > 0 ? RT / 32 : 1)) * 1024);
+        auto sgpr = [](uint32_t x) -> uint32_t { return (uint32_t)__builtin_amdgcn_readfirstlane((int)x); };
         int d_s = 0;
-        uint32_t d_off = (uint32_t)u0 * (uint32_t)(RT * RB);
-        uint32_t d_rc = kDQ ? 0u : ((uint32_t)(b * p.QH + kvh * rep) * (uint32_t)p.QLs + (uint32_t)(u0 * RT)) * 32u;
-        const uint32_t jump_off = ((uint32_t)p.QL - (uint32_t)((nps - 1) * RT)) * (uint32_t)RB;
-        const uint32_t jump_rc = ((uint32_t)p.QLs - (uint32_t)((nps - 1) * RT)) * 32u;
+        uint32_t d_off = sgpr((uint32_t)u0 * (uint32_t)(RT * RB));
+        uint32_t d_rc = kDQ ? 0u : sgpr(((uint32_t)(b * p.QH + kvh * rep) * (uint32_t)p.QLs + (uint32_t)(u0 * RT)) * 32u);
+        const uint32_t jump_off = sgpr(((uint32_t)p.QL - (uint32_t)((nps - 1) * RT)) * (uint32_t)RB);
+        const uint32_t jump_rc = sgpr(((uint32_t)p.QLs - (uint32_t)((nps - 1) * RT)) * 32u);
         auto advance_dma = [&]() {
             if constexpr (kDQ) {
                 d_off += (uint32_t)(RT * RB);
+            } else if constexpr (ONEHEAD) {
+                d_off += (uint32_t)(RT * RB);
+                d_rc += (uint32_t)(RT * 32);
             } else {
                 const int s1 = d_s + 1;
                 const bool wrap = s1 == nps;
@@ -444,8 +468,11 @@
             static_for<NJ>([&](auto jc) { constexpr int j = decltype(jc)::value; dma_piece<j, j == 0>(rs2, voff[j], d_off, slot + IMG); });
             if constexpr (!kDQ) dma_piece<0, true>(rsc, rc_voff, d_rc, slot - wave_off + rc_dst_off);
         };
-        uint32_t sM = lds0 + wave_off, sX = sM + SLOT, sF = sM + 2 * SLOT, sD = sM + 3 * SLOT, sY = sM;
-        auto rotate_slots = [&]() { sY = sM; sM = sX; sX = sF; sF = sD; sD = sY; };
+        uint32_t ring_w = lds0 + wave_off;
+        uint32_t ring_rc = lds0 + rc_dst_off;
+        asm volatile("" : "+s"(ring_w), "+s"(ring_rc));
+        uint32_t oY = (NS - 1) * SLOT, oM = 0, oX = SLOT, oF = 2 * SLOT, oD = (NS - 1) * SLOT;
+        auto rotate_slots = [&]() { oY = oM; oM = oX; oX = oF; oF = oD; oD = oY; };
 
         constexpr bool kVLds = SH::kVLds;
         frag_t b1[ZS][KS], b2[kVLds ? 1 : ZS][kVLds ? 1 : KS];
@@ -471,11 +498,11 @@
                 dma_piece<(j & 3), (j & 3) == 0>(rsv, vo, vsoff, vimg0 + (uint32_t)(wave * 16384 + (j >> 2) * 4096));
             });
         }
-        issue_step(sM);
+        issue_step(ring_w);
         advance_dma();
-        issue_step(sX);
+        issue_step(ring_w + SLOT);
         advance_dma();
-        issue_step(sF);
+        issue_step(ring_w + 2 * SLOT);
         advance_dma();
         finish_rc();
         float nl2[ZS];
@@ -511,34 +538,60 @@
 
         typedef __attribute__((address_space(3))) const frag_t* lds_frag_p;
         typedef __attribute__((address_space(3))) s16x4* lds_tr_p;
-        const uint32_t row_lane = (uint32_t)Img::row_lane_base(lane) - wave_off;
-        const uint32_t col_lane = (uint32_t)Img::col_lane_base(lane) + (uint32_t)(esplit * EB * 64) - wave_off;
-        const uint32_t rc_lane0 = (uint32_t)(2 * IMG + r * 32 + 16 * h) - wave_off;
-        const uint32_t rc_lane1 = (uint32_t)(2 * IMG + r * 32 + 16) - wave_off;
-        auto opaque = [](uint32_t x) { asm volatile("" : "+v"(x)); return x; };
+        static_assert(SLOT % Img::kRowBytes == 0 && (KS << 5) <= Img::kRowBytes && (E / 32 << 6) <= Img::kRowBytes,
+                      "a slot base never carries into the XOR-ed bits");
+        constexpr int SB = SH::SB, NBS = SH::NBS;
+        constexpr bool kBases = SH::kBases;
         auto pin = [](auto& x) { asm volatile("" : "+v"(x)); };
-        auto read_row = [&](uint32_t ra, int g) -> frag_t {
+        auto keep = [](uint32_t& x) { if constexpr (kConstSlots) asm volatile("" : "+v"(x)); };
+        uint32_t rowb[NBS][kBases ? KS : 1];
+        uint32_t colb[NBS][kBases ? 2 * EB : 1];
+        uint32_t rcb[NBS][2];
+#pragma unroll
+        for (int bs = 0; bs < (kConstSlots ? NBS : 1); ++bs) {
+            const uint32_t s0 = lds0 + (uint32_t)(bs * SB * SLOT);
+            const uint32_t row_lane = s0 + (uint32_t)Img::row_lane_base(lane);
+            const uint32_t col_lane = s0 + (uint32_t)Img::col_lane_base(lane) + (uint32_t)(esplit * EB * 64);
+            if constexpr (kBases) {
+#pragma unroll
+                for (int ks = 0; ks < KS; ++ks) { rowb[bs][ks] = row_lane ^ (uint32_t)(ks << 5); keep(rowb[bs][ks]); }
+#pragma unroll
+                for (int j = 0; j < 2 * EB; ++j) { colb[bs][j] = col_lane ^ (uint32_t)(((j >> 1) << 6) | ((j & 1) << 5)); keep(colb[bs][j]); }
+            } else {
+                rowb[bs][0] = row_lane; keep(rowb[bs][0]);
+                colb[bs][0] = col_lane; keep(colb[bs][0]);
+            }
+            if constexpr (!kDQ) {
+                rcb[bs][0] = s0 + (uint32_t)(2 * IMG + r * 32 + 16 * h); keep(rcb[bs][0]);
+                rcb[bs][1] = s0 + (uint32_t)(2 * IMG + r * 32 + 16); keep(rcb[bs][1]);
+            }
+        }
+        auto read_row = [&](auto kc, int g) -> frag_t {
             const int prod = g / (ZT * KS), zt = (g / KS) % ZT, ks = g % KS;
-            return *(lds_frag_p)(uintptr_t)((ra ^ (uint32_t)(ks << 5)) + (uint32_t)(prod * IMG + zt * 32 * RB));
+            if constexpr (std::is_same_v<decltype(kc), uint32_t>) {
+                return *(lds_frag_p)(uintptr_t)((kc ^ (uint32_t)(ks << 5)) + (uint32_t)(prod * IMG + zt * 32 * RB));
+            } else {
+                constexpr int K = decltype(kc)::value, bs = K / SB;
+                const uint32_t imm = (uint32_t)((K % SB) * SLOT + prod * IMG + zt * 32 * RB);
+                if constexpr (kBases) return *(lds_frag_p)(uintptr_t)(rowb[bs][ks] + imm);
+                else return *(lds_frag_p)(uintptr_t)((rowb[bs][0] ^ (uint32_t)(ks << 5)) + imm);
+            }
         };
-        auto read_col = [&](uint32_t ca, int f) -> frag_t {
+        auto read_col = [&](auto kc, int f) -> frag_t {
             const int y = f / (2 * ZT * EB), kk = (f / EB) % (2 * ZT), eb = f % EB;
             const int img = kDQ ? 0 : (y == 0 ? IMG : 0);
-            const s16x4 a = __builtin_amdgcn_ds_read_tr16_b64_v4i16((lds_tr_p)(uintptr_t)((ca ^ (uint32_t)(eb << 6)) + (uint32_t)(img + 16 * kk * RB)));
-            const s16x4 c = __builtin_amdgcn_ds_read_tr16_b64_v4i16((lds_tr_p)(uintptr_t)((ca ^ (uint32_t)((eb << 6) | 32)) + (uint32_t)(img + (16 * kk + 8) * RB)));
-            typedef short s16x8 __attribute__((ext_vector_type(8)));
-            const s16x8 v8 = {a[0], a[1], a[2], a[3], c[0], c[1], c[2], c[3]};
-            return __builtin_bit_cast(frag_t, v8);
-        };
-        auto read_row_b = [&](const uint32_t (&rb)[KS], int g) -> frag_t {
-            const int prod = g / (ZT * KS), zt = (g / KS) % ZT, ks = g % KS;
-            return *(lds_frag_p)(uintptr_t)(rb[ks] + (uint32_t)(prod * IMG + zt * 32 * RB));
-        };
-        auto read_col_b = [&](const uint32_t (&cb)[2 * EB], int f) -> frag_t {
-            const int y = f / (2 * ZT * EB), kk = (f / EB) % (2 * ZT), eb = f % EB;
-            const int img = kDQ ? 0 : (y == 0 ? IMG : 0);
-            const s16x4 a = __builtin_amdgcn_ds_read_tr16_b64_v4i16((lds_tr_p)(uintptr_t)(cb[2 * eb] + (uint32_t)(img + 16 * kk * RB)));
-            const s16x4 c = __builtin_amdgcn_ds_read_tr16_b64_v4i16((lds_tr_p)(uintptr_t)(cb[2 * eb + 1] + (uint32_t)(img + (16 * kk + 8) * RB)));
+            uint32_t ca, cc, imm;
+            if constexpr (std::is_same_v<decltype(kc), uint32_t>) {
+                imm = (uint32_t)(img + 16 * kk * RB);
+                ca = kc ^ (uint32_t)(eb << 6); cc = kc ^ (uint32_t)((eb << 6) | 32);
+            } else {
+                constexpr int K = decltype(kc)::value, bs = K / SB;
+                imm = (uint32_t)((K % SB) * SLOT + img + 16 * kk * RB);
+                if constexpr (kBases) { ca = colb[bs][2 * eb]; cc = colb[bs][2 * eb + 1]; }
+                else { ca = colb[bs][0] ^ (uint32_t)(eb << 6); cc = colb[bs][0] ^ (uint32_t)((eb << 6) | 32); }
+            }
+            const s16x4 a = __builtin_amdgcn_ds_read_tr16_b64_v4i16((lds_tr_p)(uintptr_t)(ca + imm));
+            const s16x4 c = __builtin_amdgcn_ds_read_tr16_b64_v4i16((lds_tr_p)(uintptr_t)(cc + imm + (uint32_t)(8 * RB)));
             typedef short s16x8 __attribute__((ext_vector_type(8)));
             const s16x8 v8 = {a[0], a[1], a[2], a[3], c[0], c[1], c[2], c[3]};
             return __builtin_bit_cast(frag_t, v8);
@@ -548,7 +601,14 @@
             const int ks = b / ZS, zs = b % ZS;
             return *(lds_frag_p)(uintptr_t)((v_lane ^ (uint32_t)(ks << 5)) + (uint32_t)(zs * 32 * RB));
         };
-        auto read_rcf = [&](uint32_t rca, int zt) -> frag_t { return *(lds_frag_p)(uintptr_t)(rca + (uint32_t)(zt * 1024)); };
+        auto read_rcf = [&](auto kc, int prod, int zt) -> frag_t {
+            if constexpr (std::is_same_v<decltype(kc), uint32_t>) {
+                return *(lds_frag_p)(uintptr_t)(rcb[0][prod] + kc + (uint32_t)(zt * 1024));
+            } else {
+                constexpr int K = decltype(kc)::value;
+                return *(lds_frag_p)(uintptr_t)(rcb[K / SB][prod] + (uint32_t)((K % SB) * SLOT + zt * 1024));
+            }
+        };
 
         uint64_t vword_next = 0;
         auto vword_fetch = [&](int u) { const int w = (u * RT) >> 6; vword_next = vbits[w < kMaxMaskTiles ? w : kMaxMaskTiles - 1]; };
@@ -628,20 +688,19 @@
         }
 
         {
-            const uint32_t ra = opaque(sM + row_lane);
-            const uint32_t rca[2] = {opaque(sM + rc_lane0), opaque(sM + rc_lane1)};
+            constexpr w64_ic<0> k0{};
 #pragma unroll
             for (int prod = 0; prod < 2; ++prod)
 #pragma unroll
                 for (int zt = 0; zt < ZT; ++zt) {
                     if constexpr (!kDQ) {
-                        const frag_t rc = read_rcf(rca[prod], zt);
+                        const frag_t rc = read_rcf(k0, prod, zt);
 #pragma unroll
                         for (int zs = 0; zs < ZS; ++zs) (prod ? dA : sA)[zs][zt] = rc_tile(rc);
                     }
 #pragma unroll
                     for (int ks = 0; ks < KS; ++ks) {
-                        const frag_t a = read_row(ra, (prod * ZT + zt) * KS + ks);
+                        const frag_t a = read_row(k0, (prod * ZT + zt) * KS + ks);
 #pragma unroll
                         for (int zs = 0; zs < ZS; ++zs) {
                             f32x16& d = (prod ? dA : sA)[zs][zt];
@@ -667,23 +726,11 @@
         if constexpr (kGeneral && kDQ) vword_fetch(0);
 
         frag_t fr[RF];
-        {
-            const uint32_t ca0 = opaque(sY + col_lane);
-#pragma unroll
-            for (int f = 0; f < PF; ++f) fr[f] = read_col(ca0, f);
-        }
-
-        constexpr bool kBases = SH::kBases;
-        uint32_t cbase[2 * EB], rbase[KS];
-        auto set_cbase = [&](uint32_t slot) {
-            const uint32_t ca = opaque(slot + col_lane);
-#pragma unroll
-            for (int j = 0; j < 2 * EB; ++j) { cbase[j] = ca ^ (uint32_t)(((j >> 1) << 6) | ((j & 1) << 5)); pin(cbase[j]); }
-        };
-        if constexpr (kBases) set_cbase(sY);
-
-        using Plan = BwdW64Plan<E, KIND, kGeneral, LAG, PF, NARROW>;
-        auto iteration = [&](int u, f32x16 (&sc)[ZS][ZT], f32x16 (&dc)[ZS][ZT], f32x16 (&sn)[ZS][ZT], f32x16 (&dn)[ZS][ZT],
+#pragma unroll
+        for (int f = 0; f < PF; ++f) fr[f] = read_col(w64_ic<NS - 1>{}, f);
+
+        using Plan = BwdW64Plan<E, KIND, kGeneral, LAG, PF, NARROW, ONEHEAD, kConstSlots>;
+        auto iteration = [&](auto pc, int u, f32x16 (&sc)[ZS][ZT], f32x16 (&dc)[ZS][ZT], f32x16 (&sn)[ZS][ZT], f32x16 (&dn)[ZS][ZT],
                              u32x4 (&fw)[NYP][ZS][2 * ZT], u32x4 (&fp)[NYP][ZS][2 * ZT]) {
             constexpr Plan plan = Plan::make();
             static_assert(plan.it_end[NSLOT - 1] == Plan::NITEM, "every item placed");
@@ -697,14 +744,18 @@
                 }
                 if (__builtin_expect(step_needs_mask(t0, valid), 0)) apply_mask(sc, t0, valid);
             }
-            const uint32_t cimg = opaque(sY + col_lane);
-            const uint32_t cimg2 = opaque(sM + col_lane);
-            const uint32_t rimg = opaque(sX + row_lane);
-            uint32_t rcimg[2] = {0, 0};
-            if constexpr (!kDQ) { rcimg[0] = opaque(sX + rc_lane0); rcimg[1] = opaque(sX + rc_lane1); }
+            constexpr int POS = decltype(pc)::value;
+            constexpr int kD = (POS + NS - 1) % NS;
+            auto slot_of = [&](auto kc, uint32_t lane_base, uint32_t off) {
+                if constexpr (kConstSlots) return kc;
+                else { uint32_t a = lane_base + off; asm volatile("" : "+v"(a)); return a; }
+            };
+            const auto kY = slot_of(w64_ic<kD>{}, colb[0][0], oY);
+            const auto kM = slot_of(w64_ic<POS>{}, colb[0][0], oM);
+            const auto kX = slot_of(w64_ic<(POS + 1) % NS>{}, rowb[0][0], oX);
+            const auto kR = [&] { if constexpr (kConstSlots) return w64_ic<(POS + 1) % NS>{}; else return oX; }();
             frag_t rcf[2 * ZT];
             frag_t vb[kVLds ? SH::RFB : 1];
-            uint32_t dst = 0, soff = 0, srow = 0;
 
             auto item = [&](auto kc) {
                 constexpr int k = decltype(kc)::value, kind = plan.kind[k], n = plan.el[k];
@@ -742,15 +793,9 @@
             };
             auto read_ahead = [&](auto fc) {
                 constexpr int g = decltype(fc)::value + PF;
-                if constexpr (kBases) {
-                    if constexpr (g < NFY) fr[g % RF] = read_col_b(cbase, g);
-                    else if constexpr (g < NF) fr[g % RF] = read_row_b(rbase, g - NFY);
-                    else fr[g % RF] = read_col_b(cbase, g - NF);
-                } else {
-                    if constexpr (g < NFY) fr[g % RF] = read_col(cimg, g);
-                    else if constexpr (g < NF) fr[g % RF] = read_row(rimg, g - NFY);
-                    else fr[g % RF] = read_col(cimg2, g - NF);
-                }
+                if constexpr (g < NFY) fr[g % RF] = read_col(kY, g);
+                else if constexpr (g < NF) fr[g % RF] = read_row(kX, g - NFY);
+                else fr[g % RF] = read_col(kM, g - NF);
             };
 
             static_for<NSLOT>([&](auto ic) {
@@ -786,7 +831,7 @@
                 if constexpr (!kDQ) {
                     static_for<2 * ZT>([&](auto tc) {
                         constexpr int tq = decltype(tc)::value;
-                        if constexpr (i == Plan::rc_read_slot(tq)) rcf[tq] = read_rcf(rcimg[tq / ZT], tq % ZT);
+                        if constexpr (i == Plan::rc_read_slot(tq)) rcf[tq] = read_rcf(kR, tq / ZT, tq % ZT);
                     });
                 }
                 if constexpr (kVLds) {
@@ -795,32 +840,31 @@
                         if constexpr (i == SH::vb_slot(b) - SH::PFB) vb[b % SH::RFB] = read_vb(b);
                     });
                 }
-                if constexpr (kBases && i == 1) {
-#pragma unroll
-                    for (int ks = 0; ks < KS; ++ks) { rbase[ks] = rimg ^ (uint32_t)(ks << 5); pin(rbase[ks]); }
-                }
-                if constexpr (kBases && i == NY + 1) set_cbase(sM);
-                if constexpr (i == Plan::BAR_SLOT + 1) {
-                    dst = sD;
-                    soff = d_off;
-                    srow = d_rc;
-                    advance_dma();
-                    asm volatile("" : "+s"(d_off));
-                }
                 static_for<NPB>([&](auto dc_) {
                     constexpr int d = decltype(dc_)::value;
                     if constexpr (i == Plan::dma_slot(d)) {
-                        if constexpr (d < NJ) dma_piece<d, d == 0>(rs1, voff[d < NJ ? d : 0], soff, dst);
-                        else if constexpr (d < 2 * NJ) dma_piece<d - NJ, d == NJ>(rs2, voff[d < 2 * NJ ? d - NJ : 0], soff, dst + IMG);
-                        else dma_piece<0, true>(rsc, rc_voff, srow, dst - wave_off + rc_dst_off);
+                        if constexpr (kConstSlots) {
+                            if constexpr (d < NJ) dma_piece_at<d, d == 0, kD * SLOT>(rs1, voff[d < NJ ? d : 0], d_off, ring_w);
+                            else if constexpr (d < 2 * NJ) dma_piece_at<d - NJ, d == NJ, kD * SLOT + IMG>(rs2, voff[d < 2 * NJ ? d - NJ : 0], d_off, ring_w);
+                            else dma_piece_at<0, true, kD * SLOT>(rsc, rc_voff, d_rc, ring_rc);
+                        } else {
+                            if constexpr (d < NJ) dma_piece<d, d == 0>(rs1, voff[d < NJ ? d : 0], d_off, ring_w + oD);
+                            else if constexpr (d < 2 * NJ) dma_piece<d - NJ, d == NJ>(rs2, voff[d < 2 * NJ ? d - NJ : 0], d_off, ring_w + oD + IMG);
+                            else dma_piece<0, true>(rsc, rc_voff, d_rc, ring_rc + oD);
+                        }
                     }
                 });
+                if constexpr (i == Plan::dma_slot(NPB - 1)) {
+                    advance_dma();
+                    if constexpr (kDQ) asm volatile("" : "+s"(d_off));
+                    else asm volatile("" : "+s"(d_off), "+s"(d_rc));
+                }
                 movable(std::integral_constant<int, i>{});
                 __builtin_amdgcn_sched_barrier(0);
             });
-            rotate_slots();
+            if constexpr (!kConstSlots) rotate_slots();
             if constexpr (kGeneral) {
-                if constexpr (kDQ) ++c_s;
+                if constexpr (kDQ || ONEHEAD) ++c_s;
                 else { if (++c_s == nps) c_s = 0; }
             }
         };
@@ -839,28 +883,37 @@
         }
         int u = 0;
         const int n_it = n_live + 1;
-        if (n_it >= 2) {
+        static_assert(NS == 4, "the body below is written out for a ring of four");
+        if constexpr (!kConstSlots) {
             for (;;) {
-                iteration(u, sA, dA, sB, dB, fA, fB);
-                iteration(u + 1, sB, dB, sA, dA, fB, fA);
+                iteration(w64_ic<0>{}, u, sA, dA, sB, dB, fA, fB);
+                iteration(w64_ic<1>{}, u + 1, sB, dB, sA, dA, fB, fA);
                 u += 2;
                 if (u + 1 >= n_it) {
                     leave_fence();
                     break;
                 }
             }
-        }
-        if (u < n_it) {
-            iteration(u, sA, dA, sB, dB, fA, fB);
-            leave_fence();
-            ++u;
-        }
+            if (u < n_it) iteration(w64_ic<0>{}, u, sA, dA, sB, dB, fA, fB);
+        } else for (;;) {
+            iteration(w64_ic<0>{}, u, sA, dA, sB, dB, fA, fB);
+            if (__builtin_expect(u + 1 < n_it, 1)) {
+                iteration(w64_ic<1>{}, u + 1, sB, dB, sA, dA, fB, fA);
+                if (__builtin_expect(u + 2 < n_it, 1)) {
+                    iteration(w64_ic<2>{}, u + 2, sA, dA, sB, dB, fA, fB);
+                    if (__builtin_expect(u + 3 < n_it, 1)) iteration(w64_ic<3>{}, u + 3, sB, dB, sA, dA, fB, fA);
+                }
+            }
+            u += 4;
+            if (u >= n_it) break;
+        }
+        u = n_it;
+        leave_fence();
         if constexpr (kDQ && kGeneral) {
             for (; u <= n_steps; ++u) {
                 asm volatile("s_waitcnt vmcnt(%0)\n\ts_barrier" :: "n"(NPB) : "memory");
-                issue_step(sD);
+                issue_step(ring_w + (uint32_t)(((u + NS - 1) % NS) * SLOT));
                 advance_dma();
-                rotate_slots();
             }
         }
         asm volatile("s_waitcnt vmcnt(0)" ::: "memory");
@@ -913,4 +966,13 @@
     }
 }
 
+template <typename T, int E, int KIND, int MODE, int NARROW = 0>
+__global__ __launch_bounds__(256, 1) void fa_bwd_w64_kernel(const BwdParams p_arg) {
+    fa_bwd_w64_body<T, E, KIND, MODE, NARROW, false>(p_arg);
 }
+template <typename T, int E, int KIND, int MODE, int NARROW = 0>
+__global__ __launch_bounds__(256, 1) void fa_bwd_w64_mha_kernel(const BwdParams p_arg) {
+    fa_bwd_w64_body<T, E, KIND, MODE, NARROW, true>(p_arg);
+}
+
+}
```

Result: no change. 984.5 TFLOP/s (-0.0%).
